# sdmiller/cpu_tsdf

Measured on AMD Instinct MI355X. Metric: integrateCloud throughput, Scene A turntable depth frames, 640x480 -> voxel grid, higher is better.
Workload: dtype f32

## Files before the change

### cpu_tsdf_amd/capi.py

```python
import ctypes as C
import os

import numpy as np

_HERE = os.path.dirname(os.path.abspath(__file__))
PRODUCT_LIB_PATH = os.path.join(_HERE, "lib", "libtsdf_hip.so")
TEST_LIB_PATH = os.path.join(_HERE, "lib", "libtsdf_hip_test.so")
LIB_PATH = os.environ.get("TSDF_HIP_LIB_PATH") or PRODUCT_LIB_PATH

OK, E_INVALID, E_NOMEM, E_HIP, E_NODEVICE, E_UNSUPPORTED, E_IO = range(7)
ALIGN_NO_POINTS, ALIGN_RANK_DEFICIENT = 7, 8
XFORM_PCL_SSE, XFORM_LEFT_TO_RIGHT = 0, 1
LAYOUT_AUTO, LAYOUT_F32W, LAYOUT_PACKED = 0, 1, 2
COLOR_RGB, COLOR_RGB_NORMALIZED, COLOR_LAB = 0, 1, 2


class TsdfParams(C.Structure):

    _fields_ = [
        ("res", C.c_int32 * 3),
        ("size", C.c_float * 3),
        ("max_dist_pos", C.c_float),
        ("max_dist_neg", C.c_float),
        ("max_weight", C.c_float),
        ("min_sensor_dist", C.c_float),
        ("max_sensor_dist", C.c_float),
        ("fx", C.c_double),
        ("fy", C.c_double),
        ("cx", C.c_double),
        ("cy", C.c_double),
        ("image_width", C.c_int32),
        ("image_height", C.c_int32),
        ("integrate_color", C.c_int32),
        ("xform_order", C.c_int32),
        ("z_begin", C.c_int32),
        ("z_end", C.c_int32),
        ("halo", C.c_int32),
        ("device", C.c_int32),
        ("layout", C.c_int32),
        ("color_mode", C.c_int32),
    ]


class TsdfVolMeta(C.Structure):

    _fields_ = [
        ("max_cell_size", C.c_float * 3),
        ("is_empty", C.c_int32),
        ("weight_by_depth", C.c_int32),
        ("weight_by_variance", C.c_int32),
        ("global_transform", C.c_double * 16),
    ]


BLOCK_FN = C.CFUNCTYPE(C.c_int, C.c_void_p, C.c_int, C.c_int, C.c_int, C.c_int, C.POINTER(C.c_float),
                       C.POINTER(C.c_float), C.POINTER(C.c_uint8))
HEADER_FN = C.CFUNCTYPE(C.c_int, C.c_void_p, C.POINTER(TsdfParams), C.POINTER(TsdfVolMeta))


class TsdfHipError(RuntimeError):
    def __init__(self, code, where, detail=""):
        self.code = code
        super().__init__(f"{where}: tsdf_hip error {code} ({detail})")


_lib = None

_f32p = C.POINTER(C.c_float)
_u8p = C.POINTER(C.c_uint8)
_u32p = C.POINTER(C.c_uint32)
_u64p = C.POINTER(C.c_uint64)
_f64p = C.POINTER(C.c_double)

SIGNATURES = {
    "tsdf_hip_default_params": (None, [C.POINTER(TsdfParams)]),
    "tsdf_hip_create": (C.c_int, [C.POINTER(TsdfParams), C.POINTER(C.c_void_p)]),
    "tsdf_hip_create_multi": (C.c_int, [C.POINTER(TsdfParams), C.POINTER(C.c_int32), C.c_int, C.POINTER(C.c_void_p)]),
    "tsdf_hip_slab_count": (C.c_int, [C.c_void_p]),
    "tsdf_hip_slab_info": (C.c_int, [C.c_void_p, C.c_int, C.POINTER(C.c_int32), C.POINTER(C.c_int32), C.POINTER(C.c_int32),
                                    C.POINTER(C.c_int32)]),
    "tsdf_hip_load_multi": (C.c_int, [C.c_char_p, C.POINTER(TsdfParams), C.POINTER(C.c_int32), C.c_int, C.POINTER(C.c_void_p),
                                     C.POINTER(TsdfParams), C.POINTER(TsdfVolMeta)]),
    "tsdf_hip_host_alloc": (C.c_int, [C.c_size_t, C.POINTER(C.c_void_p)]),
    "tsdf_hip_host_free": (C.c_int, [C.c_void_p]),
    "tsdf_hip_reset": (C.c_int, [C.c_void_p]),
    "tsdf_hip_destroy": (C.c_int, [C.c_void_p]),
    "tsdf_hip_set_stream": (C.c_int, [C.c_void_p, C.c_void_p]),
    "tsdf_hip_synchronize": (C.c_int, [C.c_void_p]),
    "tsdf_hip_integrate": (C.c_int, [C.c_void_p, _f32p, _u8p, _f32p, _u64p]),
    "tsdf_hip_integrate_async": (C.c_int, [C.c_void_p, _f32p, _u8p, _f32p]),
    "tsdf_hip_integrate_device": (C.c_int, [C.c_void_p, C.c_void_p, C.c_void_p, _f32p, _u64p]),
    "tsdf_hip_organize": (C.c_int, [C.c_void_p, _f32p, C.c_size_t, _u8p, C.c_size_t, C.c_size_t, C.c_float, C.c_int,
                                    _f64p, _f32p, _u8p, _u64p]),
    "tsdf_hip_integrate_staged": (C.c_int, [C.c_void_p, _f32p, _u64p]),
    "tsdf_hip_set_weighting": (C.c_int, [C.c_void_p, C.c_int, C.c_int]),
    "tsdf_hip_frame_begin": (C.c_int, [C.c_void_p, C.POINTER(_f32p), C.POINTER(_u8p)]),
    "tsdf_hip_frame_commit": (C.c_int, [C.c_void_p, _f32p]),
    "tsdf_hip_last_count_detail": (C.c_int, [C.c_void_p, _u64p]),
    "tsdf_hip_last_read_detail": (C.c_int, [C.c_void_p, _u64p]),
    "tsdf_hip_march_timing": (C.c_int, [C.c_void_p, _f32p, _u64p]),
    "tsdf_hip_march_stats": (C.c_int, [C.c_void_p, _u64p]),
    "tsdf_hip_raycast": (C.c_int, [C.c_void_p, _f32p, _f32p, C.c_int, _f32p]),
    "tsdf_hip_raycast_camera": (C.c_int, [C.c_void_p, _f32p, _f32p, C.c_int, _f64p, _f32p]),
    "tsdf_hip_raycast_begin": (C.c_int, [C.c_void_p, _f32p, _f32p, C.c_int, C.c_void_p]),
    "tsdf_hip_raycast_advance": (C.c_int, [C.c_void_p, _f32p, _f32p, C.c_int, C.c_int, C.c_int, C.c_void_p, C.c_void_p]),
    "tsdf_hip_raycast_advance_list": (C.c_int, [C.c_void_p, _f32p, _f32p, C.c_int, C.c_int, C.c_int, C.c_void_p, C.c_size_t]),
    "tsdf_hip_render_halo": (C.c_int, [C.POINTER(TsdfParams)]),
    "tsdf_hip_reference_cull_is_noop": (C.c_int, [C.POINTER(TsdfParams)]),
    "tsdf_hip_alloc_probe": (C.c_int, [C.c_void_p, _f32p, C.POINTER(C.c_int32)]),
    "tsdf_hip_sample": (C.c_int, [C.c_void_p, _f32p, C.c_size_t, _f32p, _f32p, _f32p, _u8p]),
    "tsdf_hip_lookup_rgb": (C.c_int, [C.c_void_p, _f32p, C.c_size_t, _u8p, _u8p]),
    "tsdf_hip_align_system": (C.c_int, [C.c_void_p, _f32p, C.c_size_t, _f64p, C.c_float, C.c_float, _f64p, _u8p, _f32p]),
    "tsdf_hip_align_system_device": (C.c_int, [C.c_void_p, C.c_void_p, C.c_size_t, _f64p, C.c_float, C.c_float, _f64p]),
    "tsdf_hip_align": (C.c_int, [C.c_void_p, _f32p, C.c_size_t, _f64p, C.c_float, C.c_float, C.c_int, C.c_double, _f64p,
                                 C.POINTER(C.c_int32), _f64p]),
    "tsdf_hip_align_stats": (C.c_int, [C.c_void_p, _u64p]),
    "tsdf_hip_march": (C.c_int, [C.c_void_p, C.c_float, C.c_int, _u64p]),
    "tsdf_hip_march_fetch": (C.c_int, [C.c_void_p, _f32p, _u8p, _u64p]),
    "tsdf_hip_march_fetch_device": (C.c_int, [C.c_void_p, C.c_void_p, C.c_void_p, C.c_void_p]),
    "tsdf_hip_mesh_cleanup": (C.c_int, [C.c_int, _f32p, C.c_uint64, _u32p, C.c_uint64, C.c_float, C.c_int, _u8p, _u64p]),
    "tsdf_hip_march_cleanup": (C.c_int, [C.c_void_p, C.c_float, C.c_int, _u64p]),
    "tsdf_hip_mesh_cleanup_stats": (C.c_int, [_u64p]),
    "tsdf_hip_mesh_flatten": (C.c_int, [C.c_int, _f32p, C.c_uint64, _u32p, C.c_uint64, C.c_float, _u32p, _u32p, _u64p, _u32p, _u64p]),
    "tsdf_hip_march_flatten": (C.c_int, [C.c_void_p, C.c_float, _u64p, _u64p]),
    "tsdf_hip_march_fetch_indexed": (C.c_int, [C.c_void_p, _f32p, _u8p, _u32p, _u64p]),
    "tsdf_hip_mesh_flatten_stats": (C.c_int, [_u64p]),
    "tsdf_hip_occupied": (C.c_int, [C.c_void_p, C.POINTER(C.c_int32), _u64p]),
    "tsdf_hip_occupied_fetch": (C.c_int, [C.c_void_p, C.POINTER(C.c_int32), _f32p, _f32p, _u8p]),
    "tsdf_hip_occupied_fetch_device": (C.c_int, [C.c_void_p, C.c_void_p, C.c_void_p, C.c_void_p, C.c_void_p]),
    "tsdf_hip_occupied_stats": (C.c_int, [C.c_void_p, _u64p]),
    "tsdf_hip_occupied_timing": (C.c_int, [C.c_void_p, _f32p]),
    "tsdf_hip_download": (C.c_int, [C.c_void_p] + [C.c_int] * 6 + [_f32p, _f32p, _u8p]),
    "tsdf_hip_upload": (C.c_int, [C.c_void_p] + [C.c_int] * 6 + [_f32p, _f32p, _u8p]),
    "tsdf_hip_download_color_state": (C.c_int, [C.c_void_p, C.c_int, C.c_int, C.c_int, _f32p]),
    "tsdf_hip_get_planes_device": (C.c_int, [C.c_void_p, C.c_int, C.c_int, C.c_void_p, C.c_void_p, C.c_void_p]),
    "tsdf_hip_set_planes_device": (C.c_int, [C.c_void_p, C.c_int, C.c_int, C.c_void_p, C.c_void_p, C.c_void_p]),
    "tsdf_hip_device_planes": (C.c_int, [C.c_void_p, C.POINTER(C.c_void_p), C.POINTER(C.c_void_p),
                                          C.POINTER(C.c_void_p), C.POINTER(C.c_int64),
                                          C.POINTER(C.c_int32), C.POINTER(C.c_int32)]),
    "tsdf_hip_layout": (C.c_int, [C.c_void_p]),
    "tsdf_hip_centers": (C.c_int, [C.c_void_p, C.c_int, _f32p]),
    "tsdf_hip_save": (C.c_int, [C.c_void_p, C.c_char_p, C.POINTER(TsdfVolMeta)]),
    "tsdf_hip_save_blocks": (C.c_int, [C.POINTER(TsdfParams), C.POINTER(TsdfVolMeta), C.c_char_p, BLOCK_FN, C.c_void_p]),
    "tsdf_hip_load_blocks": (C.c_int, [C.c_char_p, C.POINTER(TsdfParams), HEADER_FN, BLOCK_FN, C.c_void_p]),
    "tsdf_hip_load": (C.c_int, [C.c_char_p, C.POINTER(TsdfParams), C.POINTER(C.c_void_p), C.POINTER(TsdfParams),
                                C.POINTER(TsdfVolMeta)]),
    "tsdf_hip_error_string": (C.c_char_p, [C.c_int]),
    "tsdf_hip_last_error": (C.c_char_p, []),
    "tsdf_hip_device_count": (C.c_int, []),
    "tsdf_hip_abi_version": (C.c_int, []),
    "tsdf_hip_download_variance_state": (C.c_int, [C.c_void_p] + [C.c_int] * 6 + [_f32p, C.POINTER(C.c_int32)]),
    "tsdf_hip_upload_variance_state": (C.c_int, [C.c_void_p] + [C.c_int] * 6 + [_f32p, C.POINTER(C.c_int32)]),
    "tsdf_hip_set_reference_cull": (C.c_int, [C.c_void_p, _f32p]),
    "tsdf_hip_integrate_device2": (C.c_int, [C.c_void_p, C.c_void_p, C.c_void_p, _f32p, _f32p, C.c_void_p, C.c_void_p, _f32p, _f32p,
                                             _u64p, C.POINTER(C.c_int32)]),
    "tsdf_hip_set_frame_pairing": (C.c_int, [C.c_void_p, C.c_int]),
    "tsdf_hip_reference_cull_planes": (C.c_int, [C.POINTER(TsdfParams), _f64p, _f32p]),
    "tsdf_hip_last_launch_info": (C.c_int, [C.c_void_p, C.POINTER(C.c_int32)]),
    "tsdf_hip_multi_render_stats": (C.c_int, [C.c_void_p, _u64p]),
    "tsdf_hip_multi_link_stats": (C.c_int, [C.c_void_p, _u64p]),
    "tsdf_hip_multi_timing": (C.c_int, [C.c_void_p, C.c_int]),
    "tsdf_hip_multi_kernel_ms": (C.c_int, [C.c_void_p, C.c_int, _f32p, C.POINTER(C.c_int32)]),
}

TEST_SIGNATURES = {
    "tsdf_hip_selftest_checksum": (C.c_int, [C.c_void_p, _u64p]),
    "tsdf_hip_selftest_occupancy_mc": (C.c_int, [C.POINTER(C.c_int)]),
    "tsdf_hip_selftest_div_count": (C.c_int, [_f32p, C.POINTER(C.c_uint32), _f32p, _u8p, C.c_size_t]),
    "tsdf_hip_selftest_cvt_pk_u8": (C.c_int, [_f32p, C.c_size_t, C.POINTER(C.c_uint32)]),
    "tsdf_hip_selftest_rgb2lab": (C.c_int, [_u8p, C.c_size_t, _f32p]),
    "tsdf_hip_selftest_lab2rgb": (C.c_int, [_f32p, C.c_size_t, C.POINTER(C.c_uint32)]),
    "tsdf_hip_selftest_struct_oob": (C.c_int, [_f32p, C.c_int, C.c_int, C.c_int, C.c_int, C.POINTER(C.c_int32), C.POINTER(C.c_uint32), C.c_int]),
    "tsdf_hip_selftest_div_f32": (C.c_int, [_f32p, _f32p, _f32p, C.c_size_t]),
    "tsdf_hip_selftest_div_f64": (C.c_int, [_f64p, _f64p, _f64p, C.c_size_t]),
    "tsdf_hip_selftest_project": (C.c_int, [C.c_void_p, _f32p, C.c_size_t, C.POINTER(C.c_int32), C.POINTER(C.c_int32), _u8p]),
    "tsdf_hip_selftest_containing": (C.c_int, [C.c_void_p, _f32p, C.c_size_t, C.POINTER(C.c_int32)]),
    "tsdf_hip_selftest_sweep": (C.c_int, [C.c_void_p, _u64p, _u64p]),
    "tsdf_hip_selftest_read_sweep": (C.c_int, [C.c_void_p, C.c_int, _u64p, _u64p]),
    "tsdf_hip_set_tuning": (C.c_int, [C.c_char_p, C.c_int]),
    "tsdf_hip_selftest_block_flags": (C.c_int, [C.POINTER(TsdfParams), _f32p, C.c_int, C.c_int, _u8p]),
    "tsdf_hip_selftest_row_intervals": (C.c_int, [C.POINTER(TsdfParams), _f32p, _f32p, C.POINTER(C.c_uint32)]),
    "tsdf_hip_selftest_index_box": (C.c_int, [C.POINTER(TsdfParams), _f32p, C.POINTER(C.c_int32), C.POINTER(C.c_int32)]),
# ... 123 lines not shown
```

### cpu_tsdf_amd/csrc/tsdf_common.h

```cpp
#pragma once

#include <hip/hip_runtime.h>
#include <stdint.h>
#include <cmath>
#include <string>
#include <vector>

#include "tsdf_hip.h"

struct tsdf_hip_pipeline;
struct tsdf_hip_multi;

struct tsdf_hip_volume {
  tsdf_hip_multi *multi = nullptr;
  tsdf_params p;
  int device = 0;
  int nx = 0, ny = 0, nz = 0;
  int z_begin = 0, z_end = 0;
  int z_first = 0;
  int nz_alloc = 0;
  int64_t pitch = 0;
  int levels[3] = {0, 0, 0};
  float *d = nullptr, *w = nullptr;
  uint32_t *rgb = nullptr;
  uint8_t *k8 = nullptr;
  float *cn[4] = {nullptr, nullptr, nullptr, nullptr};
  float *lab_lut = nullptr;
  float4 *lab_img = nullptr;
  float *vm = nullptr;
  int32_t *vn = nullptr;
  int expf_fused_r = 0;
  float alloc_probe_ms[8] = {-1.f, -1.f, -1.f, -1.f, -1.f, -1.f, -1.f, -1.f};
  int alloc_tried = 0, alloc_chosen = 0;
  int packed = 0;
  unsigned kmax = 0;
  int weight_by_depth = 0, weight_by_variance = 0;
  float *ctr[3] = {nullptr, nullptr, nullptr};
  std::vector<float> h_ctr[3];
  float *frame_depth = nullptr;
  uint32_t *frame_bgra = nullptr;
  char *bounce = nullptr;
  hipEvent_t bounce_ev[2] = {nullptr, nullptr};
  bool bounce_busy[2] = {false, false};
  unsigned bounce_turn = 0;
  double *cam64 = nullptr;
  tsdf_hip_pipeline *pipe = nullptr;
  int frame_staged = 0;
  uint8_t *band = nullptr;
  int band_fx = 0, band_fy = 0;
  bool band_exact = false;
  int rest_state = 0;
  uint32_t rest_bits = 0;
  unsigned long long last_implied = 0, last_read_bytes = 0;
  bool last_implied_on = false;
  uint8_t *live = nullptr;
  size_t live_cap = 0;
  uint32_t *row_iv = nullptr;
  size_t row_iv_cap = 0;
  bool ctr_increasing[3] = {false, false, false};
  unsigned long long *counter = nullptr;
  unsigned long long last_observed = 0, last_changed_bytes = 0;
  bool ref_cull = false;
  float cull_planes[24] = {0};
  int last_launch[4] = {0, 0, 0, 0};
  bool pair_pending = false;
  bool pair_fused = false;
  unsigned long long pair_first_observed = 0, pair_first_changed = 0, pair_first_implied = 0, pair_first_read = 0;
  int count_slots = 0;
  bool count_ran = false;
  hipStream_t stream = nullptr;
  float *mc_verts = nullptr;
  uint8_t *mc_rgb = nullptr;
  uint64_t *mc_cell = nullptr;
  uint64_t mc_ntri = 0;
  size_t mc_cap = 0;
  bool mc_has_rgb = false;
  uint64_t *mc_keys = nullptr, *mc_vals = nullptr;
  size_t mc_cells_cap = 0;
  uint8_t *mc_need = nullptr;
  size_t mc_need_cap = 0;
  hipEvent_t mc_ev[4] = {nullptr, nullptr, nullptr, nullptr};
  float mc_ms[3] = {0.f, 0.f, 0.f};
  uint64_t mc_ncells = 0;
  uint64_t mc_d_bytes = 0;
  bool mc_skipped = false;
  hipEvent_t align_ev[2] = {nullptr, nullptr};
  uint64_t align_stats[4] = {0, 0, 0, 0};
  void *scratch = nullptr;
  size_t scratch_bytes = 0;
};

void tsdf_multi_free(tsdf_hip_volume *v);
int tsdf_multi_reset(tsdf_handle h);
int tsdf_multi_synchronize(tsdf_handle h);
int tsdf_multi_set_weighting(tsdf_handle h, int by_depth, int by_variance);
int tsdf_multi_set_reference_cull(tsdf_handle h, const float planes[24]);
int tsdf_multi_variance_block(tsdf_handle h, bool down, int x0, int y0, int z0, int nx, int ny, int nz, float *M, int32_t *nsample);
int tsdf_multi_integrate(tsdf_handle h, const float *depth, const uint8_t *bgra, const float T[12], uint64_t *n_observed,
                         bool asynchronous);
int tsdf_multi_integrate_device(tsdf_handle h, const float *d_depth, const uint32_t *d_bgra, const float T[12],
                                uint64_t *n_observed);
int tsdf_multi_organize(tsdf_handle h, const float *xyz, size_t xyz_stride, const uint8_t *bgra, size_t bgra_stride, size_t n,
                        float cloud_units, int zero_nans, const double world_to_cam[12], float *depth_out, uint8_t *bgra_out,
                        uint64_t *n_valid);
int tsdf_multi_integrate_staged(tsdf_handle h, const float T[12], uint64_t *n_observed);
int tsdf_multi_last_count_detail(tsdf_handle h, uint64_t out[2]);
int tsdf_multi_last_read_detail(tsdf_handle h, uint64_t out[3]);
int tsdf_multi_block(tsdf_handle h, bool down, int x0, int y0, int z0, int nx, int ny, int nz, float *d, float *w, uint8_t *rgb);
int tsdf_multi_sample(tsdf_handle h, const float *xyz, size_t n, float *val, float *grad, float *hess, uint8_t *ok);
int tsdf_multi_align_system(tsdf_handle h, const float *xyz, size_t n, const double vol_from_src[12], float min_weight, float r_max,
                            double out[29], uint8_t *used, float *xyz_vol);
int tsdf_multi_lookup_rgb(tsdf_handle h, const float *xyz, size_t n, uint8_t *rgb, uint8_t *found);
int tsdf_multi_raycast(tsdf_handle h, const float rot[9], const float origin[3], int downsample, const double *inv, float *out);
int tsdf_multi_march(tsdf_handle h, float w_min, int color_mode, uint64_t *n_tri);
int tsdf_multi_march_fetch(tsdf_handle h, float *verts, uint8_t *rgb, uint64_t *cell);
int tsdf_multi_march_timing(tsdf_handle h, float ms[3], uint64_t *n_cells);
int tsdf_multi_march_stats(tsdf_handle h, uint64_t out[4]);
tsdf_handle tsdf_multi_first(tsdf_handle h);
int tsdf_multi_flush(tsdf_handle h);
int tsdf_multi_set_frame_pairing(tsdf_handle h, int on);
int tsdf_multi_integrate_device2(tsdf_handle h, const float *da, const uint32_t *ca, const float TA[12], const float *planes_a, const float *db,
                                 const uint32_t *cb, const float TB[12], const float *planes_b, uint64_t *n_observed, int32_t *fused);
#define TSDF_NOT_ON_MULTI(h, what)                                                                          \
  do {                                                                                                      \
    if ((h) && (h)->multi) {                                                                                \
      tsdf_set_error(what " works on ONE slab handle; this handle is a multi-GPU set (tsdf_hip_create_multi)"); \
      return TSDF_HIP_E_UNSUPPORTED;                                                                        \
    }                                                                                                       \
  } while (0)

int tsdf_integrate_launch(tsdf_handle h, const float *d_depth, const uint32_t *d_bgra, const float T[12], bool count);
int tsdf_integrate_collect(tsdf_handle h, uint64_t *n_observed);
int tsdf_integrate_launch2(tsdf_handle h, const float *dA, const uint32_t *cA, const float TA[12], const float *planesA,
                           const float *dB, const uint32_t *cB, const float TB[12], const float *planesB, bool count, bool *fused);
int tsdf_integrate_collect2(tsdf_handle h, uint64_t n_observed[2]);

#define TSDF_MAX_SLABS 64
#define TSDF_RAY_FIN_INTS 9
unsigned tsdf_ray_list_share(int64_t n_rays, int rank, int world);
int tsdf_ray_list_begin(tsdf_handle s, const float rot[9], const float origin[3], int downsample, int rank, int world,
                        int32_t *d_list, unsigned *count);
int tsdf_ray_list_advance(tsdf_handle s, const float rot[9], const float origin[3], int downsample, int rank, int world,
                          int32_t *d_list, unsigned count, unsigned *d_incomplete);
int tsdf_ray_list_route(tsdf_handle s, const int32_t *d_list, unsigned count, int n_slab, const int *z_end,
                        unsigned *d_counters, int32_t *d_outbox, int32_t *d_finbox);
int tsdf_ray_deliver(tsdf_handle s, const int32_t *d_fin, unsigned count, float *d_out, int64_t n_pix, const double *inv);

void tsdf_set_error(const std::string &msg);
int tsdf_hip_fail(hipError_t e, const char *what, const char *file, int line);

#define TSDF_HIP_TRY(expr)                                              \
  do {                                                                  \
    hipError_t _e = (expr);                                             \
    if (_e != hipSuccess) return tsdf_hip_fail(_e, #expr, __FILE__, __LINE__); \
  } while (0)

struct TsdfDeviceScope {
  int prev = -1;
  hipError_t err;
  explicit TsdfDeviceScope(int dev) {
    err = hipGetDevice(&prev);
    if (err != hipSuccess || prev == dev)
      prev = -1;
    else
      err = hipSetDevice(dev);
  }
  ~TsdfDeviceScope() {
    if (prev >= 0) (void)hipSetDevice(prev);
  }
  TsdfDeviceScope(const TsdfDeviceScope &) = delete;
  TsdfDeviceScope &operator=(const TsdfDeviceScope &) = delete;
};
#define TSDF_ON_DEVICE(dev)          \
  TsdfDeviceScope _device_scope(dev); \
  TSDF_HIP_TRY(_device_scope.err)
int tsdf_pipeline_flush(tsdf_hip_volume *v);
#define TSDF_ENTER(h)                                  \
  TSDF_ON_DEVICE((h)->device);                         \
  if ((h)->pair_pending) {                             \
    const int _rc_flush = tsdf_pipeline_flush(h);      \
    if (_rc_flush) return _rc_flush;                   \
  }

void tsdf_build_centers(int res, float size, std::vector<float> &out, int *levels);
static inline void tsdf_lab_curve(float lut[256]) {
  for (int v = 0; v < 256; ++v) {
    float f = ((float)v / 255.);
    if (f > 0.0405)
      f = std::pow(((f + 0.055) / 1.055), 2.4);
    else
      f /= 12.92;
    f *= 100;
    lut[v] = f;
  }
}

static inline uint8_t tsdf_u8_of_float(float v) {
  const int i = (v > -2147483904.f && v < 2147483648.f) ? (int)v : (int)0x80000000;
  return (uint8_t)(i & 255);
}
static inline uint32_t tsdf_lab2rgb_host(float L, float A, float B) {
  float Y = (L + 16) / 116.;
  float X = A / 500. + Y;
  float Z = Y - (B / 200.);
  if (std::pow((double)X, 3.0) > 0.008856) X = std::pow((double)X, 3.0); else X = (X - 16 / 116.) / 7.787;
  if (std::pow((double)Y, 3.0) > 0.008856) Y = std::pow((double)Y, 3.0); else Y = (Y - 16 / 116.) / 7.787;
  if (std::pow((double)Z, 3.0) > 0.008856) Z = std::pow((double)Z, 3.0); else Z = (Z - 16 / 116.) / 7.787;
  X *= 95.047;
  Y *= 100.;
  Z *= 108.883;
  X /= 100;
  Y /= 100;
  Z /= 100;
  float rf = X * +3.2406 + Y * -1.5372 + Z * -0.4986;
  float gf = X * -0.9689 + Y * +1.8758 + Z * +0.0415;
  float bf = X * +0.0557 + Y * -0.2040 + Z * +1.0570;
  if (rf > 0.0031308) rf = 1.055 * std::pow(static_cast<double>(rf), 1. / 2.4) - 0.055; else rf *= 12.92;
  if (gf > 0.0031308) gf = 1.055 * std::pow(static_cast<double>(gf), 1. / 2.4) - 0.055; else gf *= 12.92;
  if (bf > 0.0031308) bf = 1.055 * std::pow(static_cast<double>(bf), 1. / 2.4) - 0.055; else bf *= 12.92;
  return (uint32_t)tsdf_u8_of_float(rf * 255) | ((uint32_t)tsdf_u8_of_float(gf * 255) << 8) | ((uint32_t)tsdf_u8_of_float(bf * 255) << 16);
}
void tsdf_lab2rgb_host_many(const float *L, const float *A, const float *B, size_t n, uint32_t *out);
int tsdf_lab_exact_colors(tsdf_hip_volume *v, const int64_t *d_idx, size_t n, uint32_t *host_rgb, bool write_plane);

static inline float tsdf_node_size(const tsdf_params &p, int axis) {
  const int r = p.res[0];
  const bool cubic_pow2 = r > 0 && (r & (r - 1)) == 0 && p.res[1] == r && p.res[2] == r;
  return cubic_pow2 ? p.size[0] : p.size[axis];
}
int tsdf_ensure_scratch(tsdf_hip_volume *v, size_t bytes);
int tsdf_to_host(tsdf_hip_volume *v, void *dst, const void *dev_src, size_t bytes);
int tsdf_to_device(tsdf_hip_volume *v, void *dev_dst, const void *src, size_t bytes);
void tsdf_pipeline_destroy(tsdf_hip_volume *v);

struct TsdfTuning {
  int rows_per_block;
  int blocks_per_cu;
  int fast_projection;
  int mc_flush_at;
  int mc_skip;
  int cull;
  int vol_chunk;
  int plain_kernel;
  int alloc_tries;
  int allin;
  int refcull_plain;
  int live_log2tx;
  int zfast;
  int fuse2;
  int implied_d;
  int pipe;
  int lab_chunk;
};
const TsdfTuning &tsdf_tuning();
int tsdf_vol_chunk();

struct PlaneView {
  const float *d, *w;
  const uint32_t *rgb;
  const uint8_t *k8;
  float wmax;
  unsigned kmax;
  int packed;
};

static inline PlaneView tsdf_plane_view(const tsdf_hip_volume *v) {
  return PlaneView{v->d, v->w, v->rgb, v->k8, v->p.max_weight, v->kmax, v->packed};
}

static __device__ __forceinline__ float tsdf_decode_w(unsigned k, float wmax) {
  const float kf = (float)k;
  return kf > wmax ? wmax : kf;
}

static __device__ __forceinline__ bool tsdf_encode_w(float w, float wmax, unsigned kmax, unsigned &k) {
  if (w == wmax) {
    k = kmax;
    return true;
  }
  if (w >= 0.f && w < (float)kmax && w == floorf(w)) {
    k = (unsigned)w;
    return true;
  }
  k = 0;
  return false;
}

static __device__ __forceinline__ float tsdf_load_w(const PlaneView &v, int64_t i) {
  if (!v.packed) return v.w[i];
  const unsigned k = v.rgb ? (v.rgb[i] >> 24) : (unsigned)v.k8[i];
  return tsdf_decode_w(k, v.wmax);
}

static __device__ __forceinline__ uint32_t tsdf_load_rgb(const PlaneView &v, int64_t i) {
  return v.rgb[i] & 0xffffffu;
}

static inline __host__ __device__ int64_t tsdf_index(int64_t pitch, int ny, int z_first, int x, int y,
                                                      int zg) {
  return ((int64_t)(zg - z_first) * ny + y) * pitch + x;
}
```

### cpu_tsdf_amd/csrc/tsdf_core.hip

```cpp
#include <math.h>

#include <string>
#include <stdlib.h>
#include <stdio.h>

#include <algorithm>
#include <thread>
#include <string.h>

#include <mutex>

#include "tsdf_common.h"
#include "tsdf_occupied.h"
#include "tsdf_meshpost.h"
#ifdef TSDF_HIP_TEST_HOOKS
#include "tsdf_hip_test.h"
#endif

static thread_local std::string g_last_error;

void tsdf_set_error(const std::string &msg) { g_last_error = msg; }

int tsdf_hip_fail(hipError_t e, const char *what, const char *file, int line) {
  char buf[512];
  snprintf(buf, sizeof buf, "%s:%d: %s -> %s", file, line, what, hipGetErrorString(e));
  g_last_error = buf;
  (void)hipGetLastError();
  return e == hipErrorOutOfMemory ? TSDF_HIP_E_NOMEM : TSDF_HIP_E_HIP;
}

extern "C" const char *tsdf_hip_last_error(void) { return g_last_error.c_str(); }

extern "C" const char *tsdf_hip_error_string(int code) {
  switch (code) {
    case TSDF_HIP_OK: return "ok";
    case TSDF_HIP_E_INVALID: return "invalid argument";
    case TSDF_HIP_E_NOMEM: return "out of device memory";
    case TSDF_HIP_E_HIP: return "HIP runtime error";
    case TSDF_HIP_E_NODEVICE: return "no HIP device";
    case TSDF_HIP_E_UNSUPPORTED: return "unsupported";
    case TSDF_HIP_E_IO: return "file error";
    case TSDF_HIP_ALIGN_NO_POINTS: return "alignment: no point passed the gate";
    case TSDF_HIP_ALIGN_RANK_DEFICIENT: return "alignment: the cloud does not constrain all six freedoms";
  }
  return "unknown";
}

static int env_int(const char *name, int dflt) {
  const char *e = getenv(name);
  return (e && *e) ? atoi(e) : dflt;
}

static TsdfTuning &tuning_storage() {
  static TsdfTuning t = {std::max(1, env_int("TSDF_HIP_ROWS_PER_BLOCK", 64)),
                         std::max(1, env_int("TSDF_HIP_BLOCKS_PER_CU", 8)),
                         env_int("TSDF_HIP_FAST_PROJECTION", -1), env_int("TSDF_HIP_MC_FLUSH_AT", 512), env_int("TSDF_HIP_MC_SKIP", 1),
                         env_int("TSDF_HIP_CULL", 1), std::max(1, env_int("TSDF_HIP_VOL_CHUNK", 256)),
                         env_int("TSDF_HIP_PLAIN_KERNEL", 0), env_int("TSDF_HIP_ALLOC_TRIES", 3), env_int("TSDF_HIP_ALLIN", 1),
                         env_int("TSDF_HIP_REFCULL_PLAIN", 0), env_int("TSDF_HIP_LIVE_LOG2TX", 5), env_int("TSDF_HIP_ZFAST", 1), env_int("TSDF_HIP_FUSE2", 1), env_int("TSDF_HIP_IMPLIED_D", 1),
                         env_int("TSDF_HIP_PIPE", 1), std::max(1, env_int("TSDF_HIP_LAB_CHUNK", 16 << 20))};
  return t;
}

const TsdfTuning &tsdf_tuning() { return tuning_storage(); }

int tsdf_vol_chunk() {
  const int live = env_int("TSDF_HIP_VOL_CHUNK", 0);
  return live > 0 ? live : tsdf_tuning().vol_chunk;
}

#ifdef TSDF_HIP_TEST_HOOKS
extern "C" int tsdf_hip_set_tuning(const char *name, int value) {
  if (!name) return TSDF_HIP_E_INVALID;
  TsdfTuning &t = tuning_storage();
  const std::string n(name);
  if (n == "rows_per_block")
    t.rows_per_block = std::max(1, value);
  else if (n == "blocks_per_cu")
    t.blocks_per_cu = std::max(1, value);
  else if (n == "fast_projection")
    t.fast_projection = value;
  else if (n == "mc_flush_at")
    t.mc_flush_at = value;
  else if (n == "mc_skip")
    t.mc_skip = value;
  else if (n == "cull")
    t.cull = value;
  else if (n == "vol_chunk")
    t.vol_chunk = std::max(1, value);
  else if (n == "plain_kernel")
    t.plain_kernel = value;
  else if (n == "alloc_tries")
    t.alloc_tries = std::max(1, value);
  else if (n == "allin")
    t.allin = value;
  else if (n == "refcull_plain")
    t.refcull_plain = value;
  else if (n == "fuse2")
    t.fuse2 = value;
  else if (n == "implied_d")
    t.implied_d = value;
  else if (n == "pipe")
    t.pipe = value;
  else if (n == "live_log2tx")
    t.live_log2tx = value;
  else if (n == "zfast")
    t.zfast = value;
  else if (n == "lab_chunk")
    t.lab_chunk = std::max(1, value);
  else
    return TSDF_HIP_E_INVALID;
  return TSDF_HIP_OK;
}
#endif

extern "C" int tsdf_hip_abi_version(void) { return TSDF_HIP_ABI_VERSION; }

extern "C" int tsdf_hip_host_alloc(size_t bytes, void **out) {
  if (!out || !bytes) return TSDF_HIP_E_INVALID;
  *out = nullptr;
  TSDF_HIP_TRY(hipHostMalloc(out, bytes, hipHostMallocPortable));
  return TSDF_HIP_OK;
}

extern "C" int tsdf_hip_host_free(void *p) {
  if (!p) return TSDF_HIP_OK;
  TSDF_HIP_TRY(hipHostFree(p));
  return TSDF_HIP_OK;
}

extern "C" int tsdf_hip_device_count(void) {
  int n = 0;
  if (hipGetDeviceCount(&n) != hipSuccess) {
    (void)hipGetLastError();
    return 0;
  }
  return n;
}

extern "C" void tsdf_hip_default_params(tsdf_params *p) {
  memset(p, 0, sizeof *p);
  p->res[0] = p->res[1] = p->res[2] = 512;
  p->size[0] = p->size[1] = p->size[2] = 3.0f;
  p->max_dist_pos = 0.03f;
  p->max_dist_neg = 0.03f;
  p->max_weight = 100.f;
  p->min_sensor_dist = 0.3f;
  p->max_sensor_dist = 3.0f;
  p->fx = p->fy = 525.;
  p->cx = 320;
  p->cy = 240;
  p->image_width = 640;
  p->image_height = 480;
  p->integrate_color = 0;
  p->xform_order = TSDF_XFORM_PCL_SSE;
  p->z_begin = p->z_end = 0;
  p->halo = 0;
  p->device = -1;
  p->layout = TSDF_LAYOUT_AUTO;
  p->color_mode = TSDF_COLOR_RGB;
}

static int ilog2_exact(int v) {
  if (v <= 0 || (v & (v - 1))) return -1;
  int l = 0;
  while ((1 << l) < v) ++l;
  return l;
}

void tsdf_build_centers(int res, float size, std::vector<float> &out, int *levels) {
  out.resize(res);
  const int L = ilog2_exact(res);
  *levels = L;
  if (L >= 0) {
    for (int i = 0; i < res; ++i) {
      float c = 0.f;
      float s = size;
      for (int l = L - 1; l >= 0; --l) {
        const float off = s / 4;
        c = ((i >> l) & 1) ? c + off : c - off;
        s = s / 2;
      }
      out[i] = c;
    }
  } else {
    const float off = size / 2.0;
    for (int i = 0; i < res; ++i) out[i] = (float)((i + 0.5) * size / (double)res - off);
  }
}

static __global__ void __launch_bounds__(256)
k_fill_u32(uint32_t *__restrict__ p, uint32_t value, int64_t n4 ) {
// ... 118 lines not shown
  return attr.type == hipMemoryTypeHost;
}

int tsdf_to_host(tsdf_hip_volume *v, void *dst, const void *dev_src, size_t bytes) {
  if (!bytes) return TSDF_HIP_OK;
  if (bytes >= (64u << 10) && is_pinned_host(dst)) {
    TSDF_HIP_TRY(hipMemcpyAsync(dst, dev_src, bytes, hipMemcpyDeviceToHost, v->stream));
    TSDF_HIP_TRY(hipStreamSynchronize(v->stream));
    return TSDF_HIP_OK;
  }
  int rc = bounce_ready(v);
  if (rc) return rc;
  const size_t chunks = (bytes + kBounceChunk - 1) / kBounceChunk;
  const unsigned turn = v->bounce_turn;
  v->bounce_turn += (unsigned)chunks;
  for (size_t k = 0; k <= chunks; ++k) {
    if (k < chunks) {
      const int slot = (int)((turn + k) & 1);
      if ((rc = bounce_wait(v, slot))) return rc;
      const size_t off = k * kBounceChunk, len = std::min(kBounceChunk, bytes - off);
      TSDF_HIP_TRY(hipMemcpyAsync(v->bounce + slot * kBounceChunk, (const char *)dev_src + off, len, hipMemcpyDeviceToHost,
                                  v->stream));
      TSDF_HIP_TRY(hipEventRecord(v->bounce_ev[slot], v->stream));
      v->bounce_busy[slot] = true;
    }
    if (k > 0) {
      const int slot = (int)((turn + k - 1) & 1);
      if ((rc = bounce_wait(v, slot))) return rc;
      const size_t off = (k - 1) * kBounceChunk, len = std::min(kBounceChunk, bytes - off);
      memcpy((char *)dst + off, v->bounce + slot * kBounceChunk, len);
    }
  }
  return TSDF_HIP_OK;
}

int tsdf_to_device(tsdf_hip_volume *v, void *dev_dst, const void *src, size_t bytes) {
  if (!bytes) return TSDF_HIP_OK;
  if (bytes >= (64u << 10) && is_pinned_host(src)) {
    TSDF_HIP_TRY(hipMemcpyAsync(dev_dst, src, bytes, hipMemcpyHostToDevice, v->stream));
    TSDF_HIP_TRY(hipStreamSynchronize(v->stream));
    return TSDF_HIP_OK;
  }
  int rc = bounce_ready(v);
  if (rc) return rc;
  const size_t chunks = (bytes + kBounceChunk - 1) / kBounceChunk;
  const unsigned turn = v->bounce_turn;
  v->bounce_turn += (unsigned)chunks;
  for (size_t k = 0; k < chunks; ++k) {
    const int slot = (int)((turn + k) & 1);
    if ((rc = bounce_wait(v, slot))) return rc;
    const size_t off = k * kBounceChunk, len = std::min(kBounceChunk, bytes - off);
    memcpy(v->bounce + slot * kBounceChunk, (const char *)src + off, len);
    TSDF_HIP_TRY(hipMemcpyAsync((char *)dev_dst + off, v->bounce + slot * kBounceChunk, len, hipMemcpyHostToDevice, v->stream));
    TSDF_HIP_TRY(hipEventRecord(v->bounce_ev[slot], v->stream));
    v->bounce_busy[slot] = true;
  }
  return TSDF_HIP_OK;
}

static void free_volume(tsdf_hip_volume *v) {
  if (!v) return;
  if (v->multi) tsdf_multi_free(v);
  TsdfDeviceScope scope(v->device);
  tsdf_pipeline_destroy(v);
  if (v->d) (void)hipFree(v->d);
  if (v->w) (void)hipFree(v->w);
  if (v->rgb) (void)hipFree(v->rgb);
  if (v->k8) (void)hipFree(v->k8);
  for (int c = 0; c < 4; ++c)
    if (v->cn[c]) (void)hipFree(v->cn[c]);
  if (v->vm) (void)hipFree(v->vm);
  if (v->vn) (void)hipFree(v->vn);
  if (v->lab_lut) (void)hipFree(v->lab_lut);
  if (v->lab_img) (void)hipFree(v->lab_img);
  for (int a = 0; a < 3; ++a)
    if (v->ctr[a]) (void)hipFree(v->ctr[a]);
  if (v->frame_depth) (void)hipFree(v->frame_depth);
  if (v->bounce) (void)hipHostFree(v->bounce);
  for (int i = 0; i < 2; ++i)
    if (v->bounce_ev[i]) (void)hipEventDestroy(v->bounce_ev[i]);
  if (v->cam64) (void)hipFree(v->cam64);
  if (v->live) (void)hipFree(v->live);
  if (v->row_iv) (void)hipFree(v->row_iv);
  if (v->band) (void)hipFree(v->band);
  if (v->counter) (void)hipFree(v->counter);
  if (v->mc_verts) (void)hipFree(v->mc_verts);
  if (v->mc_rgb) (void)hipFree(v->mc_rgb);
  if (v->mc_cell) (void)hipFree(v->mc_cell);
  if (v->mc_keys) (void)hipFree(v->mc_keys);
  if (v->mc_vals) (void)hipFree(v->mc_vals);
  if (v->mc_need) (void)hipFree(v->mc_need);
  for (int i = 0; i < 4; ++i)
    if (v->mc_ev[i]) (void)hipEventDestroy(v->mc_ev[i]);
  for (int i = 0; i < 2; ++i)
    if (v->align_ev[i]) (void)hipEventDestroy(v->align_ev[i]);
  if (v->scratch) (void)hipFree(v->scratch);
  delete v;
}

struct PlaneSet {
  float *d = nullptr, *w = nullptr;
  uint32_t *rgb = nullptr;
  uint8_t *k8 = nullptr;
};

static __global__ void __launch_bounds__(256)
k_probe_rmw(uint4 *__restrict__ a, uint4 *__restrict__ b, uint4 *__restrict__ c, int64_t n4, unsigned zero) {
  typedef unsigned v4u __attribute__((ext_vector_type(4)));
  v4u *pa = reinterpret_cast<v4u *>(a), *pb = reinterpret_cast<v4u *>(b), *pc = reinterpret_cast<v4u *>(c);
  for (int64_t i = (int64_t)blockIdx.x * blockDim.x + threadIdx.x; i < n4; i += (int64_t)gridDim.x * blockDim.x) {
    v4u x = __builtin_nontemporal_load(pa + i);
    x ^= zero;
    __builtin_nontemporal_store(x, pa + i);
    if (b) {
      v4u y = __builtin_nontemporal_load(pb + i);
      y ^= zero;
      __builtin_nontemporal_store(y, pb + i);
    }
    if (c) {
      v4u z = __builtin_nontemporal_load(pc + i);
      z ^= zero;
      __builtin_nontemporal_store(z, pc + i);
    }
  }
}

static void release_planes(PlaneSet &s) {
  if (s.d) (void)hipFree(s.d);
  if (s.w) (void)hipFree(s.w);
  if (s.rgb) (void)hipFree(s.rgb);
  if (s.k8) (void)hipFree(s.k8);
  s = PlaneSet();
}

static float probe_planes(const PlaneSet &s, int64_t n, hipStream_t stream) {
  hipEvent_t e0 = nullptr, e1 = nullptr;
  if (hipEventCreate(&e0) != hipSuccess || hipEventCreate(&e1) != hipSuccess) return -1.f;
  float ms = -1.f;
  const int64_t n4 = n / 4;
  const unsigned grid = 256u * (unsigned)tsdf_tuning().blocks_per_cu;
  bool ok = true;
  for (int pass = 0; pass < 2 && ok; ++pass) {
    ok &= hipEventRecord(e0, stream) == hipSuccess;
    hipLaunchKernelGGL(k_probe_rmw, dim3(grid), dim3(256), 0, stream, (uint4 *)s.d, (uint4 *)s.w, (uint4 *)s.rgb, n4, 0u);
    ok &= hipGetLastError() == hipSuccess;
    ok &= hipEventRecord(e1, stream) == hipSuccess;
    ok &= hipEventSynchronize(e1) == hipSuccess;
    if (ok) ok &= hipEventElapsedTime(&ms, e0, e1) == hipSuccess;
  }
  (void)hipEventDestroy(e0);
  (void)hipEventDestroy(e1);
  return ok ? ms : -1.f;
}

extern "C" int tsdf_hip_reference_cull_is_noop(const tsdf_params *p) {
  if (!p || !(p->fx > 0.0) || !(p->fy > 0.0) || p->image_width <= 0 || p->image_height <= 0) return 0;
  if (!(p->max_sensor_dist > 0.f) || !(p->max_sensor_dist < 1e15f)) return 0;
  const double W = p->image_width, H = p->image_height;
  const double th = tan(1.1 * atan(0.5 * W / p->fx)) * (1.0 - 1e-5), tv = tan(1.1 * atan(0.5 * H / p->fy)) * (1.0 - 1e-5);
  if (!(th > 0.0) || !(tv > 0.0)) return 0;
  return (p->cx + 1.0) / p->fx <= th && (W - p->cx) / p->fx <= th && (p->cy + 1.0) / p->fy <= tv && (H - p->cy) / p->fy <= tv;
}

extern "C" int tsdf_hip_reference_cull_planes(const tsdf_params *p, const double trans[16], float planes[24]) {
  if (!p || !trans || !planes) return TSDF_HIP_E_INVALID;
  struct V3 { float v[3]; };
// ... 94 lines not shown
  auto bail = [&](int code) {
    free_volume(v);
    return code;
  };
#define TRY_OR_BAIL(expr)                                                  \
  do {                                                                     \
    hipError_t _e = (expr);                                                \
    if (_e != hipSuccess) return bail(tsdf_hip_fail(_e, #expr, __FILE__, __LINE__)); \
  } while (0)
  auto alloc_planes = [&](PlaneSet &s) -> hipError_t {
    hipError_t e = hipMalloc(&s.d, n * sizeof(float));
    if (e == hipSuccess && !v->packed) e = hipMalloc(&s.w, n * sizeof(float));
    if (e == hipSuccess && p->integrate_color) e = hipMalloc(&s.rgb, n * sizeof(uint32_t));
    if (e == hipSuccess && v->packed && !p->integrate_color) e = hipMalloc(&s.k8, n);
    if (e != hipSuccess) release_planes(s);
    return e;
  };
  PlaneSet best;
  TRY_OR_BAIL(alloc_planes(best));
  {
    const size_t plane_bytes = (size_t)n * (4 + (v->packed ? 0 : 4) + (p->integrate_color ? 4 : 0) + (v->packed && !p->integrate_color ? 1 : 0));
    const int tries = plane_bytes >= ((size_t)4 << 30) ? std::max(1, tsdf_tuning().alloc_tries) : 1;
    float best_ms = tries > 1 ? probe_planes(best, n, v->stream) : -1.f;
    v->alloc_probe_ms[0] = best_ms;
    v->alloc_tried = 1;
    const double swept = (double)n * (4 + (v->packed ? 0 : 4) + (p->integrate_color ? 4 : 0));
    auto rate_tbps = [&](float ms) { return ms > 0.f ? 2.0 * swept / ((double)ms * 1e9) : 0.0; };
    for (int t = 1; t < std::min(8, 2 * tries) && best_ms > 0.f && tries > 1; ++t) {
      if (rate_tbps(best_ms) >= 5.55) break;
      if (t >= tries && rate_tbps(best_ms) >= 5.15) break;
      size_t free_b = 0, total_b = 0;
      if (hipMemGetInfo(&free_b, &total_b) != hipSuccess || free_b < plane_bytes + ((size_t)2 << 30)) break;
      PlaneSet cand;
      if (alloc_planes(cand) != hipSuccess) {
        (void)hipGetLastError();
        break;
      }
      const float ms = probe_planes(cand, n, v->stream);
      v->alloc_probe_ms[t < 8 ? t : 7] = ms;
      v->alloc_tried = t + 1;
      if (ms > 0.f && ms < best_ms) {
        release_planes(best);
        best = cand;
        best_ms = ms;
        v->alloc_chosen = t;
      } else {
        release_planes(cand);
      }
    }
  }
  v->d = best.d;
  v->w = best.w;
  v->rgb = best.rgb;
  v->k8 = best.k8;
  if (rgbn)
    for (int c = 0; c < (lab ? 3 : 4); ++c) TRY_OR_BAIL(hipMalloc(&v->cn[c], n * sizeof(float)));
  if (lab) {
    float lut[256];
    tsdf_lab_curve(lut);
    TRY_OR_BAIL(hipMalloc(&v->lab_lut, sizeof lut));
    TRY_OR_BAIL(hipMemcpy(v->lab_lut, lut, sizeof lut, hipMemcpyHostToDevice));
    TRY_OR_BAIL(hipMalloc(&v->lab_img, (size_t)p->image_width * p->image_height * sizeof(float4)));
  }
  for (int a = 0; a < 3; ++a) {
    tsdf_build_centers(p->res[a], tsdf_node_size(*p, a), v->h_ctr[a], &v->levels[a]);
    v->ctr_increasing[a] = true;
    for (size_t i = 1; i < v->h_ctr[a].size(); ++i) v->ctr_increasing[a] &= v->h_ctr[a][i - 1] < v->h_ctr[a][i];
    std::vector<float> padded(v->h_ctr[a]);
    padded.resize((size_t)p->res[a] + 4, NAN);
    TRY_OR_BAIL(hipMalloc(&v->ctr[a], padded.size() * sizeof(float)));
    TRY_OR_BAIL(hipMemcpy(v->ctr[a], padded.data(), padded.size() * sizeof(float), hipMemcpyHostToDevice));
  }
  const size_t npx = (size_t)p->image_width * p->image_height;
  TRY_OR_BAIL(hipMalloc(&v->frame_depth, 2 * npx * sizeof(float)));
  v->frame_bgra = reinterpret_cast<uint32_t *>(v->frame_depth + npx);
  {
    const double cam[4] = {p->fx, p->fy, p->cx, p->cy};
    TRY_OR_BAIL(hipMalloc(&v->cam64, sizeof cam));
    TRY_OR_BAIL(hipMemcpy(v->cam64, cam, sizeof cam, hipMemcpyHostToDevice));
  }
  v->band_fx = (v->nx + 63) / 64;
  v->band_fy = (v->ny + 3) / 4;
  TRY_OR_BAIL(hipMalloc(&v->band, (size_t)v->band_fx * v->band_fy * v->nz_alloc));
  TRY_OR_BAIL(hipMalloc(&v->counter, 4096 * sizeof(unsigned long long)));
  TRY_OR_BAIL(hipMemset(v->counter, 0, 4096 * sizeof(unsigned long long)));
#undef TRY_OR_BAIL
  rc = tsdf_hip_reset(v);
  if (rc != TSDF_HIP_OK) return bail(rc);
  *out = v;
  return TSDF_HIP_OK;
}

extern "C" int tsdf_hip_reset(tsdf_handle h) {
  if (!h) return TSDF_HIP_E_INVALID;
  if (h->multi) return tsdf_multi_reset(h);
  TSDF_ENTER(h);
  const int64_t n = h->pitch * h->ny * h->nz_alloc;
  const float minus_one = -1.f;
  uint32_t bits;
  memcpy(&bits, &minus_one, 4);
  int rc = fill_u32(h, h->d, bits, n);
  if (rc) return rc;
  if (h->w) rc = fill_u32(h, h->w, 0u, n);
  if (rc) return rc;
  if (h->k8) TSDF_HIP_TRY(hipMemsetAsync(h->k8, 0, (size_t)n, h->stream));
  if (h->rgb) rc = fill_u32(h, h->rgb, 0u, n);
  if (rc) return rc;
  for (int c = 0; c < 4 && !rc; ++c)
    if (h->cn[c]) rc = fill_u32(h, h->cn[c], 0u, n);
  if (rc) return rc;
  if (h->vm) rc = fill_u32(h, reinterpret_cast<float *>(h->vm), 0u, n);
  if (!rc && h->vn) rc = fill_u32(h, reinterpret_cast<float *>(h->vn), 0u, n);
  if (rc) return rc;
  TSDF_HIP_TRY(hipMemsetAsync(h->band, 0, (size_t)h->band_fx * h->band_fy * h->nz_alloc, h->stream));
  h->band_exact = true;
  h->rest_state = 0;
  TSDF_HIP_TRY(hipStreamSynchronize(h->stream));
  return TSDF_HIP_OK;
}

extern "C" int tsdf_hip_destroy(tsdf_handle h) {
  if (!h) return TSDF_HIP_E_INVALID;
  TsdfDeviceScope scope(h->device);
  (void)hipStreamSynchronize(h->stream);
  tsdf_occupied_release(h);
  tsdf_meshpost_release(h);
  free_volume(h);
  return TSDF_HIP_OK;
}

extern "C" int tsdf_hip_set_stream(tsdf_handle h, void *hip_stream) {
  if (!h) return TSDF_HIP_E_INVALID;
  TSDF_NOT_ON_MULTI(h, "tsdf_hip_set_stream (a stream belongs to one device)");
  {
    TSDF_ENTER(h);
  }
  h->stream = (hipStream_t)hip_stream;
  return TSDF_HIP_OK;
}

extern "C" int tsdf_hip_synchronize(tsdf_handle h) {
  if (!h) return TSDF_HIP_E_INVALID;
  if (h->multi) return tsdf_multi_synchronize(h);
  TSDF_ENTER(h);
  TSDF_HIP_TRY(hipStreamSynchronize(h->stream));
  return TSDF_HIP_OK;
}

extern "C" int tsdf_hip_centers(tsdf_handle h, int axis, float *out) {
  if (!h || axis < 0 || axis > 2 || !out) return TSDF_HIP_E_INVALID;
  memcpy(out, h->h_ctr[axis].data(), h->h_ctr[axis].size() * sizeof(float));
  return TSDF_HIP_OK;
}

extern "C" int tsdf_hip_alloc_probe(tsdf_handle h, float ms[8], int32_t *chosen) {
  if (!h) return 0;
  const tsdf_hip_volume *s = h->multi ? tsdf_multi_first(h) : h;
  if (ms)
    for (int i = 0; i < 8; ++i) ms[i] = s->alloc_probe_ms[i];
  if (chosen) *chosen = s->alloc_chosen;
  return s->alloc_tried;
}

extern "C" int tsdf_hip_layout(tsdf_handle h) {
  return !h ? -1 : (h->packed ? TSDF_LAYOUT_PACKED : TSDF_LAYOUT_F32W);
}

extern "C" int tsdf_hip_device_planes(tsdf_handle h, float **d, float **w, uint32_t **rgb, int64_t *pitch,
// ... 420 lines not shown
```

### cpu_tsdf_amd/csrc/tsdf_integrate.hip

```cpp
#include <limits.h>
#include <string.h>
#include <math.h>

#include <algorithm>
#include <cmath>

#include "tsdf_common.h"
#include "tsdf_div.h"
#include "tsdf_buffer.h"
#ifdef TSDF_HIP_TEST_HOOKS
#include "tsdf_hip_test.h"
#endif

#ifndef TSDF_COLOR_PK
#define TSDF_COLOR_PK 2
#endif

typedef float f2 __attribute__((ext_vector_type(2)));
typedef float f4 __attribute__((ext_vector_type(4)));

struct IntegrateArgs {
  float m[12];
  float fxf, fyf, cxf, cyf;
  float hb_u, hb_v;
  float hb_max;
  unsigned kcap, kinc;
  int hinge_fixed;
  int neg_in_window;
  unsigned kmax;
  int wmax_is_int;
  float zmin, zmax;
  float zlo;
  float pos, neg;
  float wmax;
  float pos_over_neg;
  int W, H;
  int ny;
  int plane_rows;
  int qpr;
  int z_global0;
  int zl0;
  int log2TX, TX, TY;
  int rpb;
  unsigned bgra_off;
  int expf_fused_r;
  int ref_cull;
  float cull[24];
  int band_fx, band_fy;
  int implied_d;
  int x_abs0, y_abs0;
  int zfast;
  int64_t pitch;
};

static __device__ __forceinline__ int project_exact(const IntegrateArgs &a, const double *__restrict__ cam,
                                                    float gx, float gy, float gz) {
  const Rcp64 rz = rcp64_prepare((double)gz);
  const int u = (int)(div64((double)gx * cam[0], rz) + cam[2]);
  const int v = (int)(div64((double)gy * cam[1], rz) + cam[3]);
  const bool in = (unsigned)u < (unsigned)a.W && (unsigned)v < (unsigned)a.H;
  return in ? v * a.W + u : -1;
}

template <bool ALLIN = false>
static __device__ __forceinline__ int project_fast(const IntegrateArgs &a, float gx, float gy, float gz,
                                                   bool &ambiguous, uint32_t *margin = nullptr) {
  const float y = __builtin_amdgcn_rcpf(gz);
  const float ru = __builtin_fmaf(gx * a.fxf, y, a.cxf);
  const float rv = __builtin_fmaf(gy * a.fyf, y, a.cyf);
  const int u = (int)ru, v = (int)rv;
  if (ALLIN) {
    *margin = min(__float_as_uint(__builtin_amdgcn_fractf(ru)), __float_as_uint(__builtin_amdgcn_fractf(rv)));
    ambiguous = false;
    return (int)__umul24((unsigned)v, (unsigned)a.W) + u;
  }
  const bool cert = __builtin_amdgcn_fractf(ru) > a.hb_u && __builtin_amdgcn_fractf(rv) > a.hb_v;
  ambiguous = !cert;
  const bool in = (unsigned)u < (unsigned)a.W && (unsigned)v < (unsigned)a.H;
  return in ? (int)__umul24((unsigned)v, (unsigned)a.W) + u : -1;
}

template <int ORDER>
static __device__ __forceinline__ void project_quad_allin(const IntegrateArgs &a, const float (&m)[12], const double *__restrict__ cam,
                                                          const f4 cxv, const f4 ytv, const float (&zt)[3], int (&pix)[4],
                                                          float (&gzs)[4]) {
  const f2 cxa = {cxv.x, cxv.y}, cxb = {cxv.z, cxv.w};
  const float yt[3] = {ytv.x, ytv.y, ytv.z};
  f2 ga[3], gb[3];
#pragma unroll
  for (int q = 0; q < 3; ++q) {
    if (ORDER == TSDF_XFORM_PCL_SSE) {
      ga[q] = cxa * m[4 * q] + yt[q];
      gb[q] = cxb * m[4 * q] + yt[q];
    } else {
      ga[q] = ((cxa * m[4 * q] + yt[q]) + zt[q]) + m[4 * q + 3];
      gb[q] = ((cxb * m[4 * q] + yt[q]) + zt[q]) + m[4 * q + 3];
    }
  }
  const f2 ya = {__builtin_amdgcn_rcpf(ga[2].x), __builtin_amdgcn_rcpf(ga[2].y)};
  const f2 yb = {__builtin_amdgcn_rcpf(gb[2].x), __builtin_amdgcn_rcpf(gb[2].y)};
  const f2 cxf2 = {a.cxf, a.cxf}, cyf2 = {a.cyf, a.cyf};
  const f2 rua = __builtin_elementwise_fma(ga[0] * a.fxf, ya, cxf2), rub = __builtin_elementwise_fma(gb[0] * a.fxf, yb, cxf2);
  const f2 rva = __builtin_elementwise_fma(ga[1] * a.fyf, ya, cyf2), rvb = __builtin_elementwise_fma(gb[1] * a.fyf, yb, cyf2);
  const float ru[4] = {rua.x, rua.y, rub.x, rub.y}, rv[4] = {rva.x, rva.y, rvb.x, rvb.y};
  gzs[0] = ga[2].x, gzs[1] = ga[2].y, gzs[2] = gb[2].x, gzs[3] = gb[2].y;
  uint32_t fu[4], fv[4];
#pragma unroll
  for (int j = 0; j < 4; ++j) {
    fu[j] = __float_as_uint(__builtin_amdgcn_fractf(ru[j]));
    fv[j] = __float_as_uint(__builtin_amdgcn_fractf(rv[j]));
    pix[j] = (int)__umul24((unsigned)(int)rv[j], (unsigned)a.W) + (int)ru[j];
  }
  const uint32_t hb = __float_as_uint(a.hb_max);
  const uint32_t least = min(min(min(fu[0], fv[0]), min(min(fu[1], fv[1]), fu[2])), min(min(fv[2], fu[3]), fv[3]));
  if (!(least > hb)) {
    const float gx[4] = {ga[0].x, ga[0].y, gb[0].x, gb[0].y}, gy[4] = {ga[1].x, ga[1].y, gb[1].x, gb[1].y};
#pragma unroll
    for (int j = 0; j < 4; ++j)
      if (!(min(fu[j], fv[j]) > hb)) pix[j] = project_exact(a, cam, gx[j], gy[j], gzs[j]);
  }
}

static __device__ const uint64_t k_exp2f_tab[32] = {
    0x3ff0000000000000ull, 0x3fefd9b0d3158574ull, 0x3fefb5586cf9890full, 0x3fef9301d0125b51ull, 0x3fef72b83c7d517bull,
    0x3fef54873168b9aaull, 0x3fef387a6e756238ull, 0x3fef1e9df51fdee1ull, 0x3fef06fe0a31b715ull, 0x3feef1a7373aa9cbull,
    0x3feedea64c123422ull, 0x3feece086061892dull, 0x3feebfdad5362a27ull, 0x3feeb42b569d4f82ull, 0x3feeab07dd485429ull,
    0x3feea47eb03a5585ull, 0x3feea09e667f3bcdull, 0x3fee9f75e8ec5f74ull, 0x3feea11473eb0187ull, 0x3feea589994cce13ull,
    0x3feeace5422aa0dbull, 0x3feeb737b0cdc5e5ull, 0x3feec49182a3f090ull, 0x3feed503b23e255dull, 0x3feee89f995ad3adull,
    0x3feeff76f2fb5e47ull, 0x3fef199bdd85529cull, 0x3fef3720dcef9069ull, 0x3fef5818dcfba487ull, 0x3fef7c97337b9b5full,
    0x3fefa4afa2a490daull, 0x3fefd0765b6e4540ull};

static __device__ float tsdf_expf_glibc(float x, bool fused_r) {
  const uint32_t ix = __float_as_uint(x), abstop = (ix >> 20) & 0x7ffu;
  if (abstop >= (0x42b00000u >> 20)) {
    if (ix == 0xff800000u) return 0.f;
    if (abstop >= (0x7f800000u >> 20)) return x + x;
// ... 154 lines not shown
#endif
#ifndef TSDF_EARLY_VOXEL_LOADS
#define TSDF_EARLY_VOXEL_LOADS 2
#endif

#ifndef TSDF_KTAB
#define TSDF_KTAB 0
#endif
#ifndef TSDF_LEAN_K
#define TSDF_LEAN_K 1
#endif
#ifndef TSDF_SWAR_K
#define TSDF_SWAR_K 1
#endif
#ifndef TSDF_LEAN_BAND
#define TSDF_LEAN_BAND 1
#endif
#ifndef TSDF_AMB_UNROLL
#define TSDF_AMB_UNROLL 1
#endif
#ifndef TSDF_PROJ_F2
#define TSDF_PROJ_F2 1
#endif
struct __attribute__((aligned(16))) KEntry {
  float w;
  float y;
  float hy;
  uint32_t k1;
};
static __device__ __forceinline__ KEntry tsdf_ktab_entry(const IntegrateArgs &a, unsigned k) {
  KEntry e;
  e.w = __builtin_fminf((float)k, a.wmax);
  e.y = rcp32_prepare((float)(k + 1u)).y;
  e.hy = TSDF_COLOR_PK == 2 ? __builtin_fmaf(0.5f, e.y, -0.5f) : 0.5f * e.y;
  e.k1 = min(k << 24, a.kcap) + a.kinc;
  return e;
}
#ifndef TSDF_SKIP_FIXED_HINGE
#define TSDF_SKIP_FIXED_HINGE 1
#endif
#ifndef TSDF_EXP_NO_STORE
#define TSDF_EXP_NO_STORE 0
#endif
#ifndef TSDF_EXP_NO_GATHER
#define TSDF_EXP_NO_GATHER 0
#endif
#ifndef TSDF_EXP_NO_VLOAD
#define TSDF_EXP_NO_VLOAD 0
#endif
#if TSDF_EXP_NO_VLOAD && TSDF_EARLY_VOXEL_LOADS
#error "TSDF_EXP_NO_VLOAD declares the voxel words itself: build it with -DTSDF_EARLY_VOXEL_LOADS=0 (tools/ab_bound.sh does)"
#endif
#if !TSDF_GUARD_ON_RESULT && TSDF_EARLY_VOXEL_LOADS
#error "TSDF_GUARD_ON_RESULT=0 tests the numerator d0 * w0 + dn BEFORE unread distance words are rebuilt from the counts, and with TSDF_EARLY_VOXEL_LOADS those words have no initial value: build that A/B with -DTSDF_EARLY_VOXEL_LOADS=0"
#endif
#ifndef TSDF_GATHER_AUX
#define TSDF_GATHER_AUX 0
#endif
#ifndef TSDF_WPE_MAX
#define TSDF_WPE_MAX 8
#endif
#ifndef TSDF_NO_BAND
#define TSDF_NO_BAND 0
#endif
#ifndef TSDF_BAND_PER_WAVE
#define TSDF_BAND_PER_WAVE 1
#endif
#if TSDF_BAND_PER_WAVE
#define TSDF_BAND_DECL                                                                                     \
  __shared__ __attribute__((aligned(16))) uint8_t s_band_sets[4][1024];                                    \
  reinterpret_cast<u4 *>(&s_band_sets[0][0])[tid] = (u4){0u, 0u, 0u, 0u}
#define TSDF_BAND(i) s_band_sets[threadIdx.x >> 6][i]
#define TSDF_BAND_SYNC() ((void)0)
#define TSDF_BAND_FIRST ((int)(tid & 63u))
#define TSDF_BAND_STEP 64
#else
#define TSDF_BAND_DECL                                                          \
  __shared__ __attribute__((aligned(16))) uint8_t s_band[1024 + 64];            \
  reinterpret_cast<uint32_t *>(s_band)[tid] = 0u, s_band[1024 + (tid & 63u)] = 0
#define TSDF_BAND(i) s_band[i]
#define TSDF_BAND_SYNC() __syncthreads()
#define TSDF_BAND_FIRST ((int)tid)
#define TSDF_BAND_STEP 256
#endif
#ifndef TSDF_RECOMPUTE_PX
#define TSDF_RECOMPUTE_PX 1
#endif
#ifndef TSDF_WPE_PACKED
#define TSDF_WPE_PACKED 7
#endif
#ifndef TSDF_WPE_PACKED_COLOR
#define TSDF_WPE_PACKED_COLOR 8
#endif
#define TSDF_WPE_OF(ORDER, COLOR, FASTPROJ, COUNT, PACKED, ALLIN) \
  ((ALLIN) && !(COUNT) && (PACKED) && (COLOR) && (FASTPROJ) ? TSDF_WPE_PACKED_COLOR : (ALLIN) && !(COUNT) && ((PACKED) || !(COLOR)) ? TSDF_WPE_PACKED : TSDF_WPE_GENERAL)
#ifndef TSDF_WPE_GENERAL
#define TSDF_WPE_GENERAL 7
#endif
#ifndef TSDF_PHASE_TIMER
#define TSDF_PHASE_TIMER 0
#endif
#if TSDF_PHASE_TIMER
#define TSDF_NPHASE 16
__device__ unsigned long long g_phase[1024 * TSDF_NPHASE];
static __device__ __forceinline__ uint32_t tsdf_clock_lo() {
  uint64_t t;
  asm volatile("s_memtime %0\n\ts_waitcnt lgkmcnt(0)" : "=s"(t)::"memory");
  return (uint32_t)t;
}
#define TSDF_NACC 9
#define PT_DECL                                                   \
  uint32_t pt_acc[TSDF_NACC];                                     \
  _Pragma("unroll") for (int i_ = 0; i_ < TSDF_NACC; ++i_) asm volatile("v_mov_b32 %0, 0" : "=v"(pt_acc[i_])); \
  const unsigned pt_blk = (blockIdx.x + blockIdx.y * gridDim.x + blockIdx.z * gridDim.x * gridDim.y) & 1023u; \
  uint32_t pt_prev = tsdf_clock_lo();                             \
  const uint32_t pt_t0 = pt_prev
#define PT_MARK(k)                           \
  do {                                       \
    const uint32_t pt_now = tsdf_clock_lo(); \
    pt_acc[k] += pt_now - pt_prev;           \
    pt_prev = pt_now;                        \
  } while (0)
                    \

#define PT_MARK_OUT(k)                                                                                 \
  do {                                                                                                 \
    const uint32_t pt_now = tsdf_clock_lo();                                                           \
    if ((threadIdx.x & 63u) == 0u) atomicAdd(&g_phase[pt_blk * TSDF_NPHASE + (k)], (unsigned long long)(pt_now - pt_prev)); \
    pt_prev = pt_now;                                                                                  \
  } while (0)
#define PT_COUNT(k) pt_acc[k] += 1u
#define PT_DEP4(a_, b_, c_, d_) asm volatile("" ::"v"(a_), "v"(b_), "v"(c_), "v"(d_) : "memory")
#define PT_DEP1(a_) asm volatile("" ::"v"(a_) : "memory")
#define PT_FLUSH()                                                                                       \
  do {                                                                                                   \
    const uint32_t pt_now = tsdf_clock_lo();                                                             \
    if ((threadIdx.x & 63u) == 0u) {                                                                     \
      atomicAdd(&g_phase[pt_blk * TSDF_NPHASE + 15], (unsigned long long)(pt_now - pt_t0));              \
      _Pragma("unroll") for (int i_ = 0; i_ < TSDF_NACC; ++i_)                                           \
          atomicAdd(&g_phase[pt_blk * TSDF_NPHASE + i_], (unsigned long long)pt_acc[i_]);                \
    }                                                                                                    \
  } while (0)
#else
#define PT_DECL
#define PT_MARK(k)
#define PT_MARK_OUT(k)
#define PT_COUNT(k)
#define PT_DEP4(a_, b_, c_, d_)
#define PT_DEP1(a_)
#define PT_FLUSH()
#endif
template <int ORDER, bool COLOR, bool FASTPROJ, bool COUNT, bool PACKED, bool ALLIN = false, bool LIVE = false>
static __global__ void __launch_bounds__(256) __attribute__((amdgpu_waves_per_eu(TSDF_WPE_OF(ORDER, COLOR, FASTPROJ, COUNT, PACKED, ALLIN) < TSDF_WPE_MAX ? TSDF_WPE_OF(ORDER, COLOR, FASTPROJ, COUNT, PACKED, ALLIN) : TSDF_WPE_MAX, TSDF_WPE_MAX)))
k_integrate(const IntegrateArgs a, float *__restrict__ D, float *__restrict__ Wt, uint32_t *__restrict__ RGB,
            uint8_t *__restrict__ K8, const float *__restrict__ depth, const double *__restrict__ cam,
            const float *__restrict__ ctrx, const float *__restrict__ ctry, const float *__restrict__ ctrz,
            unsigned long long *__restrict__ n_obs, const uint8_t *__restrict__ live, uint8_t *__restrict__ band,
            const uint32_t *__restrict__ row_iv) {
  static_assert(!(ALLIN && LIVE), "the ALLIN instance knows no row intervals");
  const BlockCoords bc = tsdf_block_coords(a.zfast);
  PT_DECL;
  bool strad = false;
  if (LIVE) {
    const unsigned flag = live[bc.bx + bc.gdx * (bc.by + bc.gdy * bc.bz)];
    if (flag == 0u) return;
    strad = flag == 2u;
  }
  const unsigned tid = threadIdx.x;
#if TSDF_KTAB
  __shared__ KEntry s_tab[PACKED ? 256 : 1];
#else
  __shared__ f2 s_rcp[256];
#endif
  __shared__ f4 s_yt[256];
  constexpr bool F2 = TSDF_PROJ_F2 && ALLIN && FASTPROJ;
  constexpr bool LEAN_K1 = TSDF_LEAN_K && !TSDF_KTAB && TSDF_COLOR_PK == 2 && PACKED && COLOR;
  __shared__ f4 s_cx[F2 ? 256 : 1];
  __shared__ uint32_t s_iv[LIVE ? 256 : 1];
  TSDF_BAND_DECL;
#if TSDF_KTAB
  if (PACKED) s_tab[tid] = tsdf_ktab_entry(a, tid);
#else
  if (PACKED) {
    const KEntry e = tsdf_ktab_entry(a, tid);
    s_rcp[tid] = (f2){e.y, e.hy};
  }
#endif
  {
    const int yy = (int)bc.by * a.rpb * a.TY + (int)tid;
    {
      const float cy_ = ctry[yy < a.ny ? yy : a.ny - 1], cz_ = ctrz[a.z_global0 + (int)bc.bz];
      f4 t = {0.f, 0.f, 0.f, 0.f};
#pragma unroll
      for (int q = 0; q < 3; ++q)
        t[q] = ORDER == TSDF_XFORM_PCL_SSE ? cy_ * a.m[4 * q + 1] + (cz_ * a.m[4 * q + 2] + a.m[4 * q + 3]) : a.m[4 * q + 1] * cy_;
      s_yt[tid] = t;
    }
    if (F2) {
      const int xq_ = (int)bc.bx * a.TX + (int)(tid & (unsigned)(a.TX - 1));
      if (xq_ < a.qpr) s_cx[tid] = *reinterpret_cast<const f4 *>(ctrx + xq_ * 4);
    }
    if (LIVE && strad) s_iv[tid] = yy < a.ny ? row_iv[(int64_t)bc.bz * a.ny + yy] : 0u;
  }
  __shared__ uint8_t s_bin[PACKED ? 1024 : 1];
  if (PACKED && a.implied_d) tsdf_flags_before(a, bc, band, s_bin, tid);
  __syncthreads();
  const uint64_t quiet = PACKED && a.implied_d ? tsdf_quiet_passes(a, s_bin, tid) : 0ull;
  PT_MARK_OUT(9);
  const int tx = (int)(tid & (unsigned)(a.TX - 1));
  const int ty = (int)(tid >> a.log2TX);
  const int xq = (int)bc.bx * a.TX + tx;
  const int zl = (int)bc.bz;
  const Rcp32 rneg = rcp32_prepare(a.neg);
  unsigned cnt = 0, chg = 0, imp = 0, rdb = 0;
  const int row0 = (int)bc.by * a.rpb * a.TY;
  const int rows = min(a.rpb * a.TY, a.ny - row0);
  const int64_t e0 = ((int64_t)(a.zl0 + zl) * a.plane_rows + row0) * a.pitch;
  const unsigned span = (unsigned)rows * (unsigned)a.pitch;
  const rsrc_t rsD = make_rsrc(D + e0, span * 4u);
  const rsrc_t rsW = make_rsrc(PACKED ? D : Wt + e0, PACKED ? 0u : span * 4u);
  const rsrc_t rsC = make_rsrc(COLOR ? RGB + e0 : (uint32_t *)D, COLOR ? span * 4u : 0u);
  const rsrc_t rsK = make_rsrc(PACKED && !COLOR ? K8 + e0 : (uint8_t *)D, PACKED && !COLOR ? span : 0u);
  const unsigned npix = (unsigned)a.W * (unsigned)a.H;
  const rsrc_t rsF = make_rsrc(depth, COLOR ? a.bgra_off + npix * 4u : npix * 4u);
  const i4_rsrc rsFi = make_rsrc_2d(depth, 4u, 0xffffffffu);
  if (xq < a.qpr) {
    const int x4 = xq * 4;
    const float cz = ctrz[a.z_global0 + zl];
    const float4 cx4 = *reinterpret_cast<const float4 *>(ctrx + x4);
    const float cxs[4] = {cx4.x, cx4.y, cx4.z, cx4.w};
    float px_[4][3], zt[3];
#pragma unroll
    for (int r = 0; r < 3; ++r) {
#pragma unroll
      for (int j = 0; j < 4; ++j) px_[j][r] = cxs[j] * a.m[4 * r];
      zt[r] = ORDER == TSDF_XFORM_PCL_SSE ? cz * a.m[4 * r + 2] + a.m[4 * r + 3] : a.m[4 * r + 2] * cz;
    }
    const unsigned voff = (unsigned)(ty * (int)a.pitch + x4) * 4u;
    const unsigned row_step = (unsigned)a.TY * (unsigned)a.pitch * 4u;
#if TSDF_EARLY_VOXEL_LOADS
    bool pred_obs = true;
#endif
    for (int r = 0; r < a.rpb; ++r) {
      const int y = row0 + ty + r * a.TY;
      if (y >= a.ny) break;
      unsigned iv_lo = 0u, iv_len = 0u;
      if (LIVE && strad) {
        const uint32_t iv = s_iv[ty + r * a.TY];
        iv_lo = iv & 0xffffu, iv_len = iv >> 16;
        if (!((unsigned)(x4 + 3) - iv_lo < iv_len + 3u)) continue;
      }
      const unsigned soff = (unsigned)r * row_step;
      const f4 ytv = s_yt[ty + r * a.TY];
      const float yt[3] = {ytv.x, ytv.y, ytv.z};
#if TSDF_RECOMPUTE_PX
      float px[4][3];
      if constexpr (!F2) {
        float cxr[4] = {cxs[0], cxs[1], cxs[2], cxs[3]};
#pragma unroll
        for (int j = 0; j < 4; ++j) asm volatile("" : "+v"(cxr[j]));
#pragma unroll
        for (int q = 0; q < 3; ++q)
#pragma unroll
          for (int j = 0; j < 4; ++j) px[j][q] = cxr[j] * a.m[4 * q];
      }
#else
      const float (&px)[4][3] = px_;
#endif
      auto transform = [&](int j, int q) -> float {
        if (ORDER == TSDF_XFORM_PCL_SSE) return px[j][q] + yt[q];
        return ((px[j][q] + yt[q]) + zt[q]) + a.m[4 * q + 3];
      };
      int pix[4];
      float gzs[4];
      bool any = false, lowz = false;
      if constexpr (F2) {
        asm volatile("" ::: "memory");
        project_quad_allin<ORDER>(a, a.m, cam, s_cx[tid], ytv, zt, pix, gzs);
        PT_DEP4(pix[0], pix[1], pix[2], pix[3]);
        PT_MARK(0);
      } else {
      unsigned amb_mask = 0;
      uint32_t margin[4] = {0u, 0u, 0u, 0u};
#pragma unroll
      for (int j = 0; j < 4; ++j) {
        const float gx = transform(j, 0), gy = transform(j, 1), gz = transform(j, 2);
        const bool in = ALLIN || (gz > a.zlo && !(gz > a.zmax) && (!LIVE || !strad || (unsigned)(x4 + j) - iv_lo < iv_len));
        gzs[j] = gz;
        if (!ALLIN) lowz |= in && gz < 0x1p-14f;
        int p;
        if (FASTPROJ) {
          bool amb;
          p = project_fast<ALLIN>(a, gx, gy, gz, amb, &margin[j]);
          if (amb && in) amb_mask |= 1u << j;
        } else {
          p = project_exact(a, cam, gx, gy, in ? gz : 1.f);
        }
        pix[j] = in ? p : -1;
        any |= in;
      }
      if (!ALLIN && !any) continue;
      if (ALLIN && FASTPROJ) {
        const uint32_t hb = __float_as_uint(a.hb_max);
        if (!(min(min(margin[0], margin[1]), min(margin[2], margin[3])) > hb)) {
#pragma unroll
          for (int j = 0; j < 4; ++j)
            if (!(margin[j] > hb)) amb_mask |= 1u << j;
        }
      }
#if TSDF_AMB_UNROLL
      if (FASTPROJ && amb_mask) {
#pragma unroll
        for (int j = 0; j < 4; ++j)
          if (amb_mask >> j & 1u) pix[j] = project_exact(a, cam, transform(j, 0), transform(j, 1), transform(j, 2));
      }
#else
      while (FASTPROJ && amb_mask) {
        const int j = __builtin_ctz(amb_mask);
        amb_mask &= amb_mask - 1;
        float g[3];
#pragma unroll
        for (int q = 0; q < 3; ++q)
          g[q] = j == 0 ? transform(0, q) : j == 1 ? transform(1, q) : j == 2 ? transform(2, q) : transform(3, q);
        const int p = project_exact(a, cam, g[0], g[1], g[2]);
        if (j == 0) pix[0] = p;
        if (j == 1) pix[1] = p;
        if (j == 2) pix[2] = p;
        if (j == 3) pix[3] = p;
      }
#endif
      }
#if TSDF_EARLY_VOXEL_LOADS
      constexpr bool EARLY = PACKED;
      const bool d_read = !PACKED || !(r < 64 && (quiet >> r & 1ull));
      u4 d4;
      asm volatile("" : "=v"(d4));
      u4 w4 = {0u, 0u, 0u, 0u}, c4 = {0u, 0u, 0u, 0u};
      uint32_t k4 = 0u;
      const bool ask_early = EARLY && (TSDF_EARLY_VOXEL_LOADS != 2 || pred_obs);
      if (ask_early) {
        if (d_read) d4 = bload128(rsD, voff, soff);
        if (COLOR) c4 = bload128(rsC, voff, soff);
        if (!COLOR) k4 = bload32(rsK, voff >> 2, soff >> 2);
        if (COUNT) rdb += (d_read ? 16u : 0u) + (COLOR ? 16u : 4u);
      }
#endif
      float zs[4];
      uint32_t cs[4] = {0u, 0u, 0u, 0u};
#pragma unroll
      for (int j = 0; j < 4; ++j) {
        if (TSDF_EXP_NO_GATHER) {
          zs[j] = 1e3f + (float)(pix[j] & 1);
          cs[j] = 0x00406080u + (unsigned)pix[j];
        } else if (ALLIN) {
          zs[j] = __uint_as_float(tsdf_struct_buffer_load_u32(rsFi, pix[j], 0, 0, TSDF_GATHER_AUX));
          if (COLOR) cs[j] = tsdf_struct_buffer_load_u32(rsFi, pix[j], 0, (int)a.bgra_off, TSDF_GATHER_AUX);
        } else {
          zs[j] = __uint_as_float(bload32(rsF, (unsigned)pix[j] << 2, 0u));
          if (COLOR) cs[j] = bload32(rsF, (unsigned)pix[j] << 2, a.bgra_off);
        }
      }
      PT_MARK(1);
      PT_DEP4(zs[0], zs[1], zs[2], zs[3]);
      PT_MARK(2);
      float dn[4], raw[4];
      bool act[4];
      any = false;
      bool any_div = false;
#pragma unroll
      for (int j = 0; j < 4; ++j) {
        raw[j] = zs[j] - gzs[j];
        act[j] = (ALLIN || pix[j] >= 0) && raw[j] >= -a.neg;
        dn[j] = a.pos_over_neg;
        any |= act[j];
        if (!TSDF_LEAN_BAND) any_div |= act[j] && !(raw[j] > a.pos);
      }
      if (TSDF_LEAN_BAND) {
        if (__builtin_fminf(__builtin_fminf(raw[0], raw[1]), __builtin_fminf(raw[2], raw[3])) <= a.pos) {
#pragma unroll
          for (int j = 0; j < 4; ++j) any_div |= act[j] && !(raw[j] > a.pos);
        }
      }
      if (COLOR) asm volatile("" ::"v"(cs[0]), "v"(cs[1]), "v"(cs[2]), "v"(cs[3]));
#if TSDF_EARLY_VOXEL_LOADS
      if (EARLY) {
        if (COLOR)
          asm volatile("" ::"v"(d4), "v"(c4));
        else
          asm volatile("" ::"v"(d4), "v"(k4));
      }
      const bool asked_early = ask_early;
      pred_obs = any;
#endif
      PT_MARK(3);
      if (!any) continue;
      PT_COUNT(8);
#if TSDF_EARLY_VOXEL_LOADS == 2
      if (EARLY && !asked_early) {
        if (d_read) d4 = bload128(rsD, voff, soff);
        if (COLOR) c4 = bload128(rsC, voff, soff);
        if (!COLOR) k4 = bload32(rsK, voff >> 2, soff >> 2);
        if (COUNT) rdb += (d_read ? 16u : 0u) + (COLOR ? 16u : 4u);
      }
#endif
      if (any_div) {
#pragma unroll
        for (int j = 0; j < 4; ++j) dn[j] = raw[j] > a.pos ? a.pos_over_neg : div32_fast(raw[j], rneg);
      }
      if (lowz || !a.neg_in_window) {
        asm volatile("");
#pragma unroll
        for (int j = 0; j < 4; ++j)
          if (act[j] && !(raw[j] > a.pos)) dn[j] = raw[j] / a.neg;
      }
#if TSDF_EXP_NO_VLOAD
      const uint32_t hb_ = __float_as_uint(a.pos_over_neg);
      const u4 d4 = {hb_, hb_, hb_, hb_};
      u4 w4 = {0u, 0u, 0u, 0u}, c4 = {(unsigned)r << 24, (unsigned)r << 24, (unsigned)r << 24, (unsigned)r << 24};
      uint32_t k4 = 0u;
      const bool d_read = true;
#else
#if !TSDF_EARLY_VOXEL_LOADS
      constexpr bool EARLY = false;
      const bool d_read = !PACKED || !(r < 64 && (quiet >> r & 1ull));
      u4 d4 = {0u, 0u, 0u, 0u};
      u4 w4 = {0u, 0u, 0u, 0u}, c4 = {0u, 0u, 0u, 0u};
      uint32_t k4 = 0u;
#endif
      if (!EARLY) {
        if (d_read) d4 = bload128(rsD, voff, soff);
        if (!PACKED) w4 = bload128(rsW, voff, soff);
        if (COLOR) c4 = bload128(rsC, voff, soff);
        if (PACKED && !COLOR) k4 = bload32(rsK, voff >> 2, soff >> 2);
        if (COUNT) rdb += (d_read ? 16u : 0u) + (!PACKED ? 16u : 0u) + (COLOR ? 16u : 0u) + (PACKED && !COLOR ? 4u : 0u);
      }
#endif
      PT_MARK(4);
      if (COLOR) PT_DEP4(c4.x, c4.y, c4.z, c4.w); else PT_DEP1(k4);
      PT_MARK(5);
      uint32_t d0u[4] = {d4.x, d4.y, d4.z, d4.w};
      const uint32_t c0[4] = {c4.x, c4.y, c4.z, c4.w};
      const uint32_t w0u[4] = {w4.x, w4.y, w4.z, w4.w};
      float d0[4], w0[4];
      uint32_t kw[4];
      float dv[4], wv[4];
      uint32_t cv[4], k1[4];
#if TSDF_KTAB
      float ky[4];
#endif
      float khy[4] = {0.f, 0.f, 0.f, 0.f};
#pragma unroll
      for (int j = 0; j < 4; ++j) {
        d0[j] = __uint_as_float(d0u[j]);
        w0[j] = __uint_as_float(w0u[j]);
        kw[j] = 0u;
        k1[j] = 0u;
        if (PACKED) {
          kw[j] = COLOR ? c0[j] : (k4 << (24 - 8 * j));
#if TSDF_KTAB
          const KEntry e = s_tab[kw[j] >> 24];
          w0[j] = e.w, ky[j] = e.y, khy[j] = e.hy, k1[j] = e.k1;
#else
          if (TSDF_LEAN_K && ALLIN) {
// ... 93 lines not shown
#pragma unroll
        for (int j = 0; j < 4; ++j) {
          dv[j] = d0[j];
          wv[j] = w0[j];
          cv[j] = c0[j] & 0xffffffu;
          add_observation_ieee<COLOR>(dv[j], wv[j], cv[j], dn[j], cs[j], a.wmax);
          if (COLOR) cv[j] |= k1[j] & 0xff000000u;
        }
      }
      PT_DEP4(dv[0], dv[1], cv[0], cv[1]);
      PT_MARK(6);
      uint32_t diff_w = 0u, diff_c = 0u, k4n = 0u;
      uint32_t wn_u[4];
      const uint32_t c_before[4] = {c0[0], c0[1], c0[2], c0[3]};
      if (d_touched) {
        uint32_t diff_d = 0u, dn_u[4];
#pragma unroll
        for (int j = 0; j < 4; ++j) {
          dn_u[j] = act[j] ? __float_as_uint(dv[j]) : d0u[j];
          diff_d |= dn_u[j] ^ d0u[j];
          if (COUNT) chg += dn_u[j] != d0u[j] ? 4u : 0u;
        }
        if (diff_d && !TSDF_EXP_NO_STORE) bstore128(rsD, voff, soff, (u4){dn_u[0], dn_u[1], dn_u[2], dn_u[3]});
      }
#pragma unroll
      for (int j = 0; j < 4; ++j) {
        if (PACKED && !COLOR && !TSDF_SWAR_K) k4n |= (act[j] ? k1[j] : (kw[j] & 0xff000000u)) >> (24 - 8 * j);
        wn_u[j] = act[j] ? __float_as_uint(wv[j]) : w0u[j];
        cv[j] = act[j] ? cv[j] : c0[j];
        diff_w |= wn_u[j] ^ w0u[j];
        diff_c |= cv[j] ^ c0[j];
        cnt += act[j] ? 1u : 0u;
        if (COUNT && PACKED) imp += act[j] && !d_read ? 1u : 0u;
        if (COUNT)
          chg += (!PACKED && wn_u[j] != w0u[j] ? 4u : 0u) + (COLOR && cv[j] != c_before[j] ? 4u : 0u);
      }
      if (PACKED && !COLOR && TSDF_SWAR_K) {
        const uint32_t km2 = a.kmax * 0x00010001u;
        const uint32_t te = ((k4 & 0x00ff00ffu) | 0x01000100u) - km2, to = (((k4 >> 8) & 0x00ff00ffu) | 0x01000100u) - km2;
        const uint32_t lt = ((~te >> 8) & 0x00010001u) | (((~to >> 8) & 0x00010001u) << 8);
        const uint32_t actb = (act[0] ? 0x00000001u : 0u) | (act[1] ? 0x00000100u : 0u) | (act[2] ? 0x00010000u : 0u) | (act[3] ? 0x01000000u : 0u);
        k4n = k4 + (lt & actb);
      }
      if (COUNT && PACKED && !COLOR) chg += (unsigned)__popc(((k4n ^ k4) | ((k4n ^ k4) >> 1) | ((k4n ^ k4) >> 2) | ((k4n ^ k4) >> 3) |
                                                            ((k4n ^ k4) >> 4) | ((k4n ^ k4) >> 5) | ((k4n ^ k4) >> 6) | ((k4n ^ k4) >> 7)) & 0x01010101u);
      if (!PACKED && diff_w) bstore128(rsW, voff, soff, (u4){wn_u[0], wn_u[1], wn_u[2], wn_u[3]});
      if (TSDF_EXP_NO_STORE) {
        if ((cv[0] ^ cv[1] ^ cv[2] ^ cv[3]) == 0x12345678u) bstore32(rsD, voff, soff, cv[0] ^ diff_w);
      } else
      if (COLOR && diff_c) bstore128(rsC, voff, soff, (u4){cv[0], cv[1], cv[2], cv[3]});
      if (PACKED && !COLOR && k4n != k4) bstore32(rsK, voff >> 2, soff >> 2, k4n);
      PT_MARK(7);
    }
  }
  PT_MARK_OUT(10);
  if (!TSDF_NO_BAND && band) {
    TSDF_BAND_SYNC();
    const int lf = max(0, a.log2TX - 4), fxb = 1 << lf;
    const int yg0 = (a.y_abs0 + row0) >> 2, yg1 = (a.y_abs0 + row0 + max(rows, 1) - 1) >> 2;
    const int xc0 = (a.x_abs0 + (int)bc.bx * a.TX * 4) >> 6;
    const int n_fl = (yg1 - yg0 + 1) << lf;
    for (int i = TSDF_BAND_FIRST; i < n_fl; i += TSDF_BAND_STEP) {
      const int yg = yg0 + (i >> lf), xc = xc0 + (i & (fxb - 1));
      if (TSDF_BAND(i) && yg < a.band_fy && xc < a.band_fx) band[((int64_t)(a.zl0 + zl) * a.band_fy + yg) * a.band_fx + xc] = 1;
    }
  }
  PT_MARK_OUT(12);
  PT_FLUSH();
  if (COUNT) {
    __shared__ unsigned s_cnt, s_chg, s_imp, s_rdb;
    if (tid == 0) s_cnt = s_chg = s_imp = s_rdb = 0;
    __syncthreads();
    if (cnt) atomicAdd(&s_cnt, cnt);
    if (chg) atomicAdd(&s_chg, chg);
    if (imp) atomicAdd(&s_imp, imp);
    if (rdb) atomicAdd(&s_rdb, rdb);
    __syncthreads();
    if (tid == 0 && (s_cnt || s_rdb)) {
      const unsigned b = bc.bx + bc.by * bc.gdx + bc.bz * bc.gdx * bc.gdy;
      if (s_cnt) atomicAdd(n_obs + (b & 1023u), (unsigned long long)s_cnt);
      if (s_chg) atomicAdd(n_obs + 1024u + (b & 1023u), (unsigned long long)s_chg);
      if (s_imp) atomicAdd(n_obs + 2048u + (b & 1023u), (unsigned long long)s_imp);
      if (s_rdb) atomicAdd(n_obs + 3072u + (b & 1023u), (unsigned long long)s_rdb);
    }
  }
}

#ifndef TSDF_WPE_PIPE
#define TSDF_WPE_PIPE 8
#endif
struct PipeRow {
  float gz[4];
  uint32_t z[4];
  uint32_t k4;
  u4 d4;
};

template <int ORDER, bool COUNT>
static __global__ void __launch_bounds__(256) __attribute__((amdgpu_waves_per_eu(TSDF_WPE_PIPE < TSDF_WPE_MAX ? TSDF_WPE_PIPE : TSDF_WPE_MAX, TSDF_WPE_MAX)))
k_integrate_p(const IntegrateArgs a, float *__restrict__ D, uint8_t *__restrict__ K8, const float *__restrict__ depth,
              const double *__restrict__ cam, const float *__restrict__ ctrx, const float *__restrict__ ctry,
              const float *__restrict__ ctrz, unsigned long long *__restrict__ n_obs, uint8_t *__restrict__ band) {
  const BlockCoords bc = tsdf_block_coords(a.zfast);
  const unsigned tid = threadIdx.x;
  __shared__ f2 s_rcp[256];
  __shared__ f4 s_yt[256];
  __shared__ f4 s_cx[256];
  __shared__ uint8_t s_bin[1024];
  TSDF_BAND_DECL;
  {
    const KEntry e = tsdf_ktab_entry(a, tid);
    s_rcp[tid] = (f2){e.y, e.hy};
    const int yy = (int)bc.by * a.rpb * a.TY + (int)tid;
    const float cy_ = ctry[yy < a.ny ? yy : a.ny - 1], cz_ = ctrz[a.z_global0 + (int)bc.bz];
    f4 t = {0.f, 0.f, 0.f, 0.f};
#pragma unroll
    for (int q = 0; q < 3; ++q)
      t[q] = ORDER == TSDF_XFORM_PCL_SSE ? cy_ * a.m[4 * q + 1] + (cz_ * a.m[4 * q + 2] + a.m[4 * q + 3]) : a.m[4 * q + 1] * cy_;
    s_yt[tid] = t;
    const int xq_ = (int)bc.bx * a.TX + (int)(tid & (unsigned)(a.TX - 1));
    if (xq_ < a.qpr) s_cx[tid] = *reinterpret_cast<const f4 *>(ctrx + xq_ * 4);
  }
  if (a.implied_d) tsdf_flags_before(a, bc, band, s_bin, tid);
  __syncthreads();
  const uint64_t quiet = a.implied_d ? tsdf_quiet_passes(a, s_bin, tid) : 0ull;
  const int tx = (int)(tid & (unsigned)(a.TX - 1));
  const int ty = (int)(tid >> a.log2TX);
  const int xq = (int)bc.bx * a.TX + tx;
  const int zl = (int)bc.bz;
  const Rcp32 rneg = rcp32_prepare(a.neg);
  unsigned cnt = 0, chg = 0, imp = 0, rdb = 0;
  const int row0 = (int)bc.by * a.rpb * a.TY;
  const int rows = min(a.rpb * a.TY, a.ny - row0);
  const int64_t e0 = ((int64_t)(a.zl0 + zl) * a.plane_rows + row0) * a.pitch;
  const unsigned span = (unsigned)rows * (unsigned)a.pitch;
  const rsrc_t rsD = make_rsrc(D + e0, span * 4u);
  const rsrc_t rsK = make_rsrc(K8 + e0, span);
  const i4_rsrc rsFi = make_rsrc_2d(depth, 4u, 0xffffffffu);
  const uint32_t pbits = __float_as_uint(a.pos_over_neg);
  if (xq < a.qpr) {
    const int x4 = xq * 4;
    const float cz = ctrz[a.z_global0 + zl];
    float zt[3];
#pragma unroll
    for (int q = 0; q < 3; ++q) zt[q] = ORDER == TSDF_XFORM_PCL_SSE ? cz * a.m[4 * q + 2] + a.m[4 * q + 3] : a.m[4 * q + 2] * cz;
    const unsigned voff = (unsigned)(ty * (int)a.pitch + x4) * 4u;
    const unsigned row_step = (unsigned)a.TY * (unsigned)a.pitch * 4u;

    auto issue = [&](const int r, PipeRow &R) {
      const f4 ytv = s_yt[ty + r * a.TY];
      asm volatile("" ::: "memory");
      int pix[4];
      project_quad_allin<ORDER>(a, a.m, cam, s_cx[tid], ytv, zt, pix, R.gz);
      const unsigned soff = (unsigned)r * row_step;
      const bool d_read = !(r < 64 && (quiet >> r & 1ull));
      if (d_read)
        R.d4 = bload128(rsD, voff, soff);
      else
        asm volatile("" : "=v"(R.d4));
      R.k4 = bload32(rsK, voff >> 2, soff >> 2);
#pragma unroll
      for (int j = 0; j < 4; ++j) R.z[j] = tsdf_struct_buffer_load_u32(rsFi, pix[j], 0, 0, TSDF_GATHER_AUX);
      if (COUNT) rdb += (d_read ? 16u : 0u) + 4u;
    };

    auto consume = [&](const int r, const PipeRow &R) {
// ... 815 lines not shown
  const float a = fabsf(v);
  return nextafterf(a, INFINITY) - a;
}

struct IntegrateHost {
  IntegrateArgs a;
  float band_u, band_v;
  double fx, fy;
  int planes;
};

static IntegrateHost make_args(tsdf_handle h, const float T[12]) {
  const tsdf_params &p = h->p;
  IntegrateHost hh;
  IntegrateArgs &a = hh.a;
  for (int i = 0; i < 12; ++i) a.m[i] = T[i];
  hh.fx = p.fx;
  hh.fy = p.fy;
  a.fxf = (float)p.fx;
  a.fyf = (float)p.fy;
  {
    auto band = [](double c, int n) {
      const double q = std::max(fabs(c) + 1.0, fabs((double)n + 1.0 - c));
      const double e = q * (2.0 / 16777216.0 + 1.0 / 4194304.0) * 1.0000005 + ((double)n + 2.0) / 16777216.0 +
                       2.0 * f32_ulp((float)c) + 1e-9;
      return nextafterf((float)(1.5 * e), INFINITY);
    };
    hh.band_u = band(p.cx, p.image_width);
    hh.band_v = band(p.cy, p.image_height);
    a.cxf = (float)(p.cx + (double)hh.band_u);
    a.cyf = (float)(p.cy + (double)hh.band_v);
    a.hb_u = nextafterf(2.f * hh.band_u, INFINITY);
    a.hb_v = nextafterf(2.f * hh.band_v, INFINITY);
    a.hb_max = std::max(a.hb_u, a.hb_v);
  }
  a.zmin = p.min_sensor_dist;
  a.zlo = p.min_sensor_dist > 0.f ? nextafterf(p.min_sensor_dist, -INFINITY) : 0.f;
  a.zmax = p.max_sensor_dist;
  a.pos = p.max_dist_pos;
  a.neg = p.max_dist_neg;
  a.wmax = p.max_weight;
  a.kmax = h->kmax;
  a.kcap = h->kmax ? (h->kmax - 1u) << 24 : 0u;
  a.kinc = h->kmax ? 0x01000000u : 0u;
  a.wmax_is_int = p.max_weight == floorf(p.max_weight);
  a.pos_over_neg = p.max_dist_pos / p.max_dist_neg;
  {
    const volatile float pv = a.pos_over_neg;
    bool fixed = h->packed && a.wmax_is_int && std::isnormal(a.pos_over_neg);
    for (unsigned k = 0; fixed && k <= h->kmax; ++k) {
      const volatile float w = fminf((float)k, p.max_weight);
      const volatile float num = pv * w;
      const volatile float sum = num + pv;
      const volatile float den = w + 1.f;
      const volatile float q = sum / den;
      fixed = q == pv;
    }
    a.hinge_fixed = fixed ? 1 : 0;
  }
  a.neg_in_window = p.max_dist_neg >= 0x1p-20f && p.max_dist_neg <= 0x1p20f && p.max_dist_pos <= 0x1p20f;
  a.W = p.image_width;
  a.H = p.image_height;
  a.ny = h->ny;
  a.plane_rows = h->ny;
  a.qpr = (h->nx + 3) / 4;
  hh.planes = h->z_end - h->z_begin;
  a.z_global0 = h->z_begin;
  a.zl0 = h->z_begin - h->z_first;
  int l2 = 0;
  while ((1 << l2) < a.qpr && l2 < 8) ++l2;
  a.log2TX = l2;
  a.TX = 1 << l2;
  a.TY = 256 / a.TX;
  a.rpb = std::max(1, std::min(tsdf_tuning().rows_per_block, 256) / a.TY);
  a.rpb = std::max(1, std::min(a.rpb, (a.ny + a.TY - 1) / a.TY));
  a.pitch = h->pitch;
  a.expf_fused_r = h->expf_fused_r;
  a.ref_cull = h->ref_cull ? 1 : 0;
  for (int i = 0; i < 24; ++i) a.cull[i] = h->ref_cull ? h->cull_planes[i] : 0.f;
  a.band_fx = h->band_fx;
  a.band_fy = h->band_fy;
  a.x_abs0 = a.y_abs0 = 0;
  a.zfast = 0;
  return hh;
}

template <int ORDER>
static __global__ void __launch_bounds__(256)
k_integrate_rgbn(const IntegrateArgs a, float *__restrict__ D, float *__restrict__ Wt, uint32_t *__restrict__ RGB,
                 float *__restrict__ RN, float *__restrict__ GN, float *__restrict__ BN, float *__restrict__ IN,
                 const float *__restrict__ depth, const uint32_t *__restrict__ bgra, const double *__restrict__ cam,
                 const float *__restrict__ ctrx, const float *__restrict__ ctry, const float *__restrict__ ctrz,
                 unsigned long long *__restrict__ n_obs) {
  const int x = (int)(blockIdx.x * 256u + threadIdx.x);
  const int y = (int)blockIdx.y, zl = (int)blockIdx.z;
  bool observed = false;
  if (x < (int)a.pitch) {
    const float cx = ctrx[x], cy = ctry[y], cz = ctrz[a.z_global0 + zl];
    float g[3];
#pragma unroll
    for (int q = 0; q < 3; ++q)
      g[q] = ORDER == TSDF_XFORM_PCL_SSE ? cx * a.m[4 * q] + (cy * a.m[4 * q + 1] + (cz * a.m[4 * q + 2] + a.m[4 * q + 3]))
                                         : ((a.m[4 * q] * cx + a.m[4 * q + 1] * cy) + a.m[4 * q + 2] * cz) + a.m[4 * q + 3];
    const bool in = !(g[2] < a.zmin || g[2] > a.zmax) && g[2] > 0.f &&
                    (!a.ref_cull || reference_cull_keeps(a, cx, cy, cz));
    const int pix = in ? project_exact(a, cam, g[0], g[1], g[2]) : -1;
    if (pix >= 0) {
      const float z = depth[pix];
      float dn = z - g[2];
      if (!isnan(z) && !(dn < -a.neg)) {
        dn = dn > a.pos ? a.pos_over_neg : dn / a.neg;
        const int64_t vi = ((int64_t)(a.zl0 + zl) * a.plane_rows + y) * a.pitch + x;
        const uint32_t c = bgra[pix];
        const float r = (float)((c >> 16) & 255u), gch = (float)((c >> 8) & 255u), b = (float)(c & 255u);
        float w = Wt[vi], d = D[vi];
        const float wn = 1.f;
        const float wsum = w + wn;
        const float i = sqrtf(r * r + gch * gch + b * b);
        const float rf = r / i, gf = gch / i, bf = b / i;
        const float rn = (w * RN[vi] + wn * rf) / wsum;
        const float gn = (w * GN[vi] + wn * gf) / wsum;
        const float bn = (w * BN[vi] + wn * bf) / wsum;
        const float im = (w * IN[vi] + wn * i) / wsum;
        RN[vi] = rn;
        GN[vi] = gn;
        BN[vi] = bn;
        IN[vi] = im;
        RGB[vi] = ((uint32_t)(int)(rn * im) & 255u) | (((uint32_t)(int)(gn * im) & 255u) << 8) |
                  (((uint32_t)(int)(bn * im) & 255u) << 16);
        uint32_t unused = 0;
        add_observation_ieee<false>(d, w, unused, dn, 0u, a.wmax);
        D[vi] = d;
        Wt[vi] = w;
        observed = true;
      }
    }
  }
  if (n_obs) {
    const unsigned long long m = __ballot(observed);
    if ((threadIdx.x & 63u) == 0u && m)
      atomicAdd(n_obs + ((blockIdx.x + blockIdx.y * gridDim.x + blockIdx.z * gridDim.x * gridDim.y) & 1023u),
                (unsigned long long)__popcll(m));
  }
}

static __device__ __forceinline__ float lab_f(float t) {
  return (double)t > 0.008856 ? (float)pow((double)t, 1 / 3.) : (float)(7.787 * (double)t + (16 / 116.));
}

static __global__ void __launch_bounds__(256)
k_lab_image(const uint32_t *__restrict__ bgra, const float *__restrict__ lut, float4 *__restrict__ lab, int n) {
  const int i = (int)(blockIdx.x * 256u + threadIdx.x);
  if (i >= n) return;
  const uint32_t c = bgra[i];
  const double rf = (double)lut[(c >> 16) & 255u], gf = (double)lut[(c >> 8) & 255u], bf = (double)lut[c & 255u];
  float X = (float)(rf * 0.4124 + gf * 0.3576 + bf * 0.1805);
  float Y = (float)(rf * 0.2126 + gf * 0.7152 + bf * 0.0722);
  float Z = (float)(rf * 0.0193 + gf * 0.1192 + bf * 0.9505);
  X = (float)((double)X / 95.047);
  Y = (float)((double)Y / 100.);
  Z = (float)((double)Z / 108.883);
  X = lab_f(X);
  Y = lab_f(Y);
  Z = lab_f(Z);
  lab[i] = make_float4((116.f * Y) - 16.f, 500.f * (X - Y), 200.f * (Y - Z), 0.f);
}
// ... 225 lines not shown
    for (int r = 0; r < 3; ++r) {
      const double c = inv[3 * r] * (g[0] - t[0]) + inv[3 * r + 1] * (g[1] - t[1]) + inv[3 * r + 2] * (g[2] - t[2]);
      if (!std::isfinite(c)) return false;
      mn[r] = std::min(mn[r], c);
      mx[r] = std::max(mx[r], c);
      big = std::max(big, fabs(c));
    }
  }
  for (int a = 0; a < 3; ++a) {
    const std::vector<float> &ctr = h->h_ctr[a];
    const int n = (int)ctr.size();
    const double margin = 2.0 * (double)p.size[a] / (double)p.res[a] + 1e-5 * (big + fabs((double)p.size[a]));
    if (mx[a] + margin < (double)ctr.front() || mn[a] - margin > (double)ctr.back()) *empty = true;
    lo[a] = (int)(std::lower_bound(ctr.begin(), ctr.end(), (float)(mn[a] - margin)) - ctr.begin());
    hi[a] = (int)(std::upper_bound(ctr.begin(), ctr.end(), (float)(mx[a] + margin)) - ctr.begin()) - 1;
    if (lo[a] > 0) --lo[a];
    if (hi[a] < n - 1) ++hi[a];
    if (lo[a] > hi[a]) *empty = true;
  }
  return true;
}

static bool zlo_margin_ok(const float T[12], const tsdf_hip_volume *h) {
  double big = 0, zmin = 1e300;
  for (int k = 0; k < 8; ++k) {
    const double x = h->h_ctr[0][(k & 1) ? h->nx - 1 : 0], y = h->h_ctr[1][(k & 2) ? h->ny - 1 : 0],
                 z = h->h_ctr[2][(k & 4) ? h->z_end - 1 : h->z_begin];
    for (int r = 0; r < 3; ++r) {
      const double g = fabs((double)T[4 * r] * x) + fabs((double)T[4 * r + 1] * y) + fabs((double)T[4 * r + 2] * z) + fabs((double)T[4 * r + 3]);
      big = std::max(big, g);
    }
    zmin = std::min(zmin, (double)T[8] * x + (double)T[9] * y + (double)T[10] * z + (double)T[11]);
  }
  const double err = 8.0 * 6e-8 * big;
  const double f = std::max(fabs(h->p.fx), fabs(h->p.fy));
  return err < 1e-4 && zmin > 0.05 && f * err * (1.0 + big / zmin) / zmin < 0.05;
}

static bool reference_cull_keeps_whole_slab(const tsdf_hip_volume *h, const float *planes) {
  for (int k = 0; k < 6; ++k) {
    const float *pl = planes + 4 * k;
    double worst = -1e300, mag = 0;
    for (int c = 0; c < 8; ++c) {
      const double x = h->h_ctr[0][(c & 1) ? h->nx - 1 : 0], y = h->h_ctr[1][(c & 2) ? h->ny - 1 : 0],
                   z = h->h_ctr[2][(c & 4) ? h->z_end - 1 : h->z_begin];
      const double v = (double)pl[0] * x + (double)pl[1] * y + (double)pl[2] * z + (double)pl[3];
      if (!std::isfinite(v)) return false;
      worst = std::max(worst, v);
      mag = std::max(mag, fabs((double)pl[0] * x) + fabs((double)pl[1] * y) + fabs((double)pl[2] * z) + fabs((double)pl[3]));
    }
    if (!(worst + 8.0 * 4.0 * 5.97e-8 * mag <= 0.0)) return false;
  }
  return true;
}

static bool row_intervals_usable(const tsdf_hip_volume *h, bool planes) {
  if (h->pitch > 0xfff0 || !h->ctr_increasing[0]) return false;
  if (planes)
    for (int i = 0; i < 24; ++i)
      if (!(fabsf(h->cull_planes[i]) < 1e30f)) return false;
  return true;
}

static bool slab_all_inside(const tsdf_hip_volume *h, const float T[12]) {
  const tsdf_params &p = h->p;
  bool all_inside = true;
  for (int k = 0; k < 8 && all_inside; ++k) {
    const double x = h->h_ctr[0][(k & 1) ? h->nx - 1 : 0], y = h->h_ctr[1][(k & 2) ? h->ny - 1 : 0],
                 z = h->h_ctr[2][(k & 4) ? h->z_end - 1 : h->z_begin];
    double g[3];
    for (int r = 0; r < 3; ++r) g[r] = (double)T[4 * r] * x + (double)T[4 * r + 1] * y + (double)T[4 * r + 2] * z + (double)T[4 * r + 3];
    const double u = p.fx * g[0] / g[2] + p.cx, v = p.fy * g[1] / g[2] + p.cy;
    const double zlo = p.min_sensor_dist > 0 ? p.min_sensor_dist : 0;
    all_inside = g[2] > zlo + 1e-3 && g[2] > 1e-3 && g[2] < p.max_sensor_dist - 1e-3 && u > 1 && u < p.image_width - 2 && v > 1 &&
                 v < p.image_height - 2;
  }
  return all_inside;
}

int tsdf_integrate_launch(tsdf_handle h, const float *d_depth, const uint32_t *d_bgra, const float T[12], bool count) {
  const tsdf_params &p = h->p;
  h->count_slots = 0;
  h->count_ran = false;
  const IntegrateHost hh = make_args(h, T);
  IntegrateArgs a = hh.a;
  unsigned gx = (unsigned)((a.qpr + a.TX - 1) / a.TX);
  unsigned gy = (unsigned)((a.ny + a.rpb * a.TY - 1) / (a.rpb * a.TY));
  unsigned gz = (unsigned)hh.planes;
  if (gy > 65535u || gz > 65535u) {
    tsdf_set_error("grid too large for one launch");
    return TSDF_HIP_E_UNSUPPORTED;
  }
  const bool color = p.integrate_color != 0;
  if (color && !d_bgra) {
    tsdf_set_error("integrate_color is set but no colour image was given");
    return TSDF_HIP_E_INVALID;
  }
  if (h->weight_by_variance && (!h->vm || !h->vn || h->packed || h->cn[0])) {
    tsdf_set_error("weight_by_variance_ (hpp:203-204) needs the per-voxel M_ / nsample_ planes: F32W layout, TSDF_COLOR_RGB");
    return TSDF_HIP_E_UNSUPPORTED;
  }
  const bool rc = h->ref_cull && !reference_cull_keeps_whole_slab(h, h->cull_planes);
  const bool rc_rows = rc && !h->cn[0] && !tsdf_tuning().refcull_plain && row_intervals_usable(h, true);
  const int plain_mode = h->weight_by_depth ? 2 : h->weight_by_variance ? 4 : (rc && !rc_rows && !h->cn[0]) ? 3 : (tsdf_tuning().plain_kernel && !h->packed && !h->cn[0] ? 1 : 0);
  a.ref_cull = rc ? 1 : 0;
  if (plain_mode || h->cn[0]) h->band_exact = false;
  if (plain_mode) {
    if ((h->packed && plain_mode != 3) || h->cn[0]) {
      tsdf_set_error("weight_by_depth needs the F32W layout and TSDF_COLOR_RGB");
      return TSDF_HIP_E_UNSUPPORTED;
    }
    if (count) TSDF_HIP_TRY(hipMemsetAsync(h->counter, 0, 1024 * sizeof(unsigned long long), h->stream));
    bool pose_ok = true;
    for (int i = 0; i < 12; ++i) pose_ok &= std::isfinite(T[i]) && fabsf(T[i]) <= 1e15f;
    if (pose_ok) {
      const dim3 grid((unsigned)((h->pitch + 255) / 256), (unsigned)h->ny, gz), block(256);
      if (grid.y > 65535u) {
        tsdf_set_error("grid too large for one launch");
        return TSDF_HIP_E_UNSUPPORTED;
      }
#define LAUNCH_PLAIN(ORDER, COLOR, BYD, PK)                                                                             \
  hipLaunchKernelGGL((k_integrate_plain<ORDER, COLOR, BYD, PK>), grid, block, 0, h->stream, a, h->d, h->w, h->rgb, h->k8, \
                     h->weight_by_variance ? h->vm : nullptr, h->weight_by_variance ? h->vn : nullptr, d_depth, d_bgra,   \
                     h->cam64, h->ctr[0], h->ctr[1], h->ctr[2], count ? h->counter : nullptr)
#define LP2(ORDER, COLOR)                      \
  do {                                         \
    if (plain_mode == 2)                       \
      LAUNCH_PLAIN(ORDER, COLOR, true, false); \
    else if (h->packed)                        \
      LAUNCH_PLAIN(ORDER, COLOR, false, true); \
    else                                       \
      LAUNCH_PLAIN(ORDER, COLOR, false, false); \
  } while (0)
      if (p.xform_order == TSDF_XFORM_PCL_SSE) {
        if (color)
          LP2(TSDF_XFORM_PCL_SSE, true);
        else
          LP2(TSDF_XFORM_PCL_SSE, false);
      } else {
        if (color)
          LP2(TSDF_XFORM_LEFT_TO_RIGHT, true);
        else
          LP2(TSDF_XFORM_LEFT_TO_RIGHT, false);
      }
#undef LP2
#undef LAUNCH_PLAIN
      TSDF_HIP_TRY(hipGetLastError());
    }
    h->count_slots = count ? 1024 : 0;
    h->count_ran = pose_ok;
    return TSDF_HIP_OK;
  }
  if (h->cn[0]) {
    if (count) TSDF_HIP_TRY(hipMemsetAsync(h->counter, 0, 1024 * sizeof(unsigned long long), h->stream));
    bool pose_ok = true;
    for (int i = 0; i < 12; ++i) pose_ok &= std::isfinite(T[i]) && fabsf(T[i]) <= 1e15f;
    if (pose_ok) {
      const dim3 grid((unsigned)((h->pitch + 255) / 256), (unsigned)h->ny, gz), block(256);
      if (grid.y > 65535u) {
        tsdf_set_error("grid too large for one launch");
        return TSDF_HIP_E_UNSUPPORTED;
      }
      if (h->lab_img) {
        const int npx = p.image_width * p.image_height;
        hipLaunchKernelGGL(k_lab_image, dim3((unsigned)((npx + 255) / 256)), dim3(256), 0, h->stream, d_bgra,
                           h->lab_lut, h->lab_img, npx);
// ... 57 lines not shown
      a.rpb = std::max(1, std::min(2 * tsdf_tuning().rows_per_block, 64) / a.TY);
      gx = (unsigned)((a.qpr + a.TX - 1) / a.TX);
      gy = (unsigned)((a.ny + a.rpb * a.TY - 1) / (a.rpb * a.TY));
    }
    int lo[3], hi[3];
    bool empty = false;
    if (tsdf_tuning().cull && !all_inside && observable_index_box(h, T, lo, hi, &empty)) {
      lo[2] = std::max(lo[2], h->z_begin);
      hi[2] = std::min(hi[2], h->z_end - 1);
      if (empty || lo[2] > hi[2]) {
        nothing_observable = true;
      } else {
        const int bxv = a.TX * 4, byr = a.rpb * a.TY;
        const int bx0 = lo[0] / bxv, bx1 = hi[0] / bxv, by0 = lo[1] / byr, by1 = hi[1] / byr;
        const int x_off = bx0 * bxv, y_off = by0 * byr, z_off = lo[2] - h->z_begin;
        const int64_t e_off = (int64_t)y_off * h->pitch + x_off;
        D += e_off;
        if (Wt) Wt += e_off;
        if (RGB) RGB += e_off;
        if (K8) K8 += e_off;
        ctrx += x_off;
        ctry += y_off;
        a.qpr -= x_off / 4;
        a.ny -= y_off;
        a.x_abs0 = x_off;
        a.y_abs0 = y_off;
        a.z_global0 += z_off;
        a.zl0 += z_off;
        gx = (unsigned)(bx1 - bx0 + 1);
        gy = (unsigned)(by1 - by0 + 1);
        gz = (unsigned)(hi[2] - lo[2] + 1);
      }
    }
    if (gy > 65535u) {
      tsdf_set_error("grid too large for one launch");
      return TSDF_HIP_E_UNSUPPORTED;
    }
    if (!nothing_observable) {
      CullArgs c;
      for (int i = 0; i < 12; ++i) c.m[i] = T[i];
      c.fx = p.fx, c.fy = p.fy, c.cx = p.cx, c.cy = p.cy;
      c.zlo = p.min_sensor_dist > 0 ? p.min_sensor_dist : 0;
      c.zmax = p.max_sensor_dist;
      c.W = p.image_width, c.H = p.image_height;
      c.nx = h->nx - (int)(ctrx - h->ctr[0]), c.ny = a.ny, c.z_global0 = a.z_global0;
      c.bx_vox = a.TX * 4, c.by_rows = a.rpb * a.TY;
      c.gx = (int)gx, c.gy = (int)gy, c.gz = (int)gz;
      const int rows = std::min(a.ny, (int)gy * a.rpb * a.TY);
      a.ny = rows;
      c.ny = rows;
      RowArgs ra;
      for (int i = 0; i < 12; ++i) ra.m[i] = T[i];
      ra.fx = p.fx, ra.fy = p.fy, ra.cx = p.cx, ra.cy = p.cy;
      ra.zlo = c.zlo, ra.zmax = c.zmax;
      ra.W = c.W, ra.H = c.H;
      ra.nx = std::min(c.nx, (int)gx * a.TX * 4), ra.ny = rows, ra.nz = (int)gz, ra.z_global0 = a.z_global0;
      ra.rc = rc_rows ? 1 : 0;
      for (int i = 0; i < 24; ++i) ra.cull[i] = rc_rows ? h->cull_planes[i] : 0.f;
      const size_t nb = (size_t)gx * gy * gz, nrows = (size_t)rows * gz;
      if (nb > h->live_cap || nrows > h->row_iv_cap) {
        TSDF_HIP_TRY(hipStreamSynchronize(h->stream));
        if (nb > h->live_cap) {
          if (h->live) TSDF_HIP_TRY(hipFree(h->live));
          h->live = nullptr, h->live_cap = 0;
          TSDF_HIP_TRY(hipMalloc(&h->live, nb));
          h->live_cap = nb;
        }
        if (nrows > h->row_iv_cap) {
          if (h->row_iv) TSDF_HIP_TRY(hipFree(h->row_iv));
          h->row_iv = nullptr, h->row_iv_cap = 0;
          TSDF_HIP_TRY(hipMalloc(&h->row_iv, nrows * sizeof(uint32_t)));
          h->row_iv_cap = nrows;
        }
      }
      if (ra.nx <= TSDF_ROWS_LDS_NX)
        hipLaunchKernelGGL(k_rows<true>, dim3((unsigned)((nrows + 255) / 256)), dim3(256), 0, h->stream, ra, ctrx, ctry, h->ctr[2], h->row_iv);
      else
        hipLaunchKernelGGL(k_rows<false>, dim3((unsigned)((nrows + 255) / 256)), dim3(256), 0, h->stream, ra, ctrx, ctry, h->ctr[2], h->row_iv);
      hipLaunchKernelGGL(k_cull, dim3((unsigned)((nb + 255) / 256)), dim3(256), 0, h->stream, c, ctrx, ctry, h->ctr[2], h->row_iv, h->live);
      TSDF_HIP_TRY(hipGetLastError());
      live = h->live;
    }
  }
  if (count) TSDF_HIP_TRY(hipMemsetAsync(h->counter, 0, 4096 * sizeof(unsigned long long), h->stream));
  bool pose_ok = true;
  for (int i = 0; i < 12; ++i) pose_ok &= std::isfinite(T[i]) && fabsf(T[i]) <= 1e15f;
  const bool fastproj = fast_projection_ok(hh, p.integrate_color != 0);
  h->last_launch[0] = h->last_launch[1] = h->last_launch[2] = h->last_launch[3] = 0;
  uint8_t *band_arg = h->band_exact && ((a.rpb * a.TY) & 3) == 0 && (a.y_abs0 & 3) == 0 ? h->band : nullptr;
  if (!band_arg) h->band_exact = false;
  a.implied_d = implied_distances(h, a, band_arg != nullptr);
  h->last_implied_on = a.implied_d != 0;
  if (pose_ok && !nothing_observable) {
    const size_t frame_bytes = npx * (color ? 8 : 4);
    a.zfast = tsdf_tuning().zfast < 0 ? (frame_bytes > (3u << 20) && gx <= 65535u) : (tsdf_tuning().zfast != 0 && gx <= 65535u);
    const dim3 grid(a.zfast ? gz : gx, gy, a.zfast ? gx : gz), block(256);
    h->last_launch[0] = fastproj && allin && !live;
    h->last_launch[1] = fastproj;
    h->last_launch[2] = live ? (rc_rows ? 2 : 1) : 0;
    h->last_launch[3] = (int)std::min<uint64_t>((uint64_t)gx * gy * gz, 0x7fffffffu);
#define LAUNCH(ORDER, COLOR, FP, COUNT, PK, AI, LV)                                                                  \
  hipLaunchKernelGGL((k_integrate<ORDER, COLOR, FP, COUNT, PK, AI, LV>), grid, block, 0, h->stream, a, D, Wt, RGB, K8, \
                     d_depth, h->cam64, ctrx, ctry, h->ctr[2], h->counter, live, band_arg, h->row_iv)
#define L6(ORDER, COLOR, FP, COUNT, PK)                  \
  do {                                                   \
    if (live)                                            \
      LAUNCH(ORDER, COLOR, FP, COUNT, PK, false, true);  \
    else if (FP && allin)                                \
      LAUNCH(ORDER, COLOR, FP, COUNT, PK, FP, false);    \
    else                                                 \
      LAUNCH(ORDER, COLOR, FP, COUNT, PK, false, false); \
  } while (0)
#define L5(ORDER, COLOR, FP, COUNT)     \
  do {                                  \
    if (h->packed)                      \
      L6(ORDER, COLOR, FP, COUNT, true);  \
    else                                \
      L6(ORDER, COLOR, FP, COUNT, false); \
  } while (0)
#define L4(ORDER, COLOR, FP) \
  do {                       \
    if (count)               \
      L5(ORDER, COLOR, FP, true);  \
    else                     \
      L5(ORDER, COLOR, FP, false); \
  } while (0)
#define L2(ORDER, COLOR) \
  do {                   \
    if (fastproj)        \
      L4(ORDER, COLOR, true);  \
    else                 \
      L4(ORDER, COLOR, false); \
  } while (0)
    const bool pipe = (tsdf_tuning().pipe & (color ? 2 : 1)) && fastproj && allin && !live && h->packed && a.hinge_fixed && a.neg_in_window &&
                      a.ny % a.TY == 0;
    if (pipe) {
      h->last_launch[0] |= 0x100;
#define LAUNCH_P(ORDER, COUNT)                                                                                                           \
  do {                                                                                                                                   \
    if (color)                                                                                                                           \
      hipLaunchKernelGGL((k_integrate_pc<ORDER, COUNT>), grid, block, 0, h->stream, a, D, RGB, d_depth, h->cam64, ctrx, ctry, h->ctr[2], \
                         h->counter, band_arg);                                                                                          \
    else                                                                                                                                 \
      hipLaunchKernelGGL((k_integrate_p<ORDER, COUNT>), grid, block, 0, h->stream, a, D, K8, d_depth, h->cam64, ctrx, ctry, h->ctr[2],   \
                         h->counter, band_arg);                                                                                          \
  } while (0)
      if (p.xform_order == TSDF_XFORM_PCL_SSE) {
        if (count)
          LAUNCH_P(TSDF_XFORM_PCL_SSE, true);
        else
          LAUNCH_P(TSDF_XFORM_PCL_SSE, false);
      } else {
        if (count)
          LAUNCH_P(TSDF_XFORM_LEFT_TO_RIGHT, true);
        else
          LAUNCH_P(TSDF_XFORM_LEFT_TO_RIGHT, false);
      }
#undef LAUNCH_P
    } else if (p.xform_order == TSDF_XFORM_PCL_SSE) {
      if (color)
        L2(TSDF_XFORM_PCL_SSE, true);
      else
        L2(TSDF_XFORM_PCL_SSE, false);
    } else {
      if (color)
        L2(TSDF_XFORM_LEFT_TO_RIGHT, true);
      else
        L2(TSDF_XFORM_LEFT_TO_RIGHT, false);
    }
#undef L2
#undef L4
#undef L5
#undef L6
#undef LAUNCH
    TSDF_HIP_TRY(hipGetLastError());
#if TSDF_PHASE_TIMER
    if (const char *pf = getenv("TSDF_HIP_PHASE_FILE")) {
      TSDF_HIP_TRY(hipStreamSynchronize(h->stream));
      static unsigned long long host_ph[1024 * TSDF_NPHASE];
      TSDF_HIP_TRY(hipMemcpyFromSymbol(host_ph, HIP_SYMBOL(g_phase), sizeof host_ph));
      unsigned long long sum[TSDF_NPHASE] = {0};
      for (int i = 0; i < 1024; ++i)
        for (int k = 0; k < TSDF_NPHASE; ++k) sum[k] += host_ph[i * TSDF_NPHASE + k];
      memset(host_ph, 0, sizeof host_ph);
      TSDF_HIP_TRY(hipMemcpyToSymbol(HIP_SYMBOL(g_phase), host_ph, sizeof host_ph));
      if (FILE *f = fopen(pf, "a")) {
        fprintf(f, "{\"color\": %d, \"count\": %d, \"allin\": %d, \"live\": %d, \"packed\": %d, \"blocks\": %d, \"phase\": [", (int)color, (int)count,
                (int)(fastproj && allin && !live), (int)(live != nullptr), (int)h->packed, h->last_launch[3]);
        for (int k = 0; k < TSDF_NPHASE; ++k) fprintf(f, "%llu%s", sum[k], k + 1 < TSDF_NPHASE ? ", " : "]}\n");
        fclose(f);
      }
    }
#endif
  }
  h->count_slots = count ? 4096 : 0;
  h->count_ran = pose_ok && !nothing_observable;
  return TSDF_HIP_OK;
}

int tsdf_integrate_collect(tsdf_handle h, uint64_t *n_observed) {
  if (!h->count_slots) {
    tsdf_set_error("tsdf_integrate_collect without a counting launch");
    return TSDF_HIP_E_INVALID;
  }
  unsigned long long c[4096];
  const int slots = h->count_slots;
  TSDF_HIP_TRY(hipMemcpyAsync(c, h->counter, (size_t)slots * sizeof(unsigned long long), hipMemcpyDeviceToHost, h->stream));
  TSDF_HIP_TRY(hipStreamSynchronize(h->stream));
  unsigned long long sum = 0, changed = 0, implied = 0, read_bytes = 0;
  for (int i = 0; i < 1024; ++i) sum += c[i];
  for (int i = 1024; i < slots && i < 2048; ++i) changed += c[i];
  for (int i = 2048; i < slots && i < 3072; ++i) implied += c[i];
  for (int i = 3072; i < slots; ++i) read_bytes += c[i];
  h->last_observed = h->count_ran ? sum : 0;
  h->last_changed_bytes = h->count_ran ? changed : 0;
  h->last_implied = h->count_ran ? implied : 0;
  h->last_read_bytes = h->count_ran ? read_bytes : 0;
  h->count_slots = 0;
  if (n_observed) *n_observed = h->last_observed;
  return TSDF_HIP_OK;
}

static int launch_integrate(tsdf_handle h, const float *d_depth, const uint32_t *d_bgra, const float T[12],
                            uint64_t *n_observed) {
  const int rc = tsdf_integrate_launch(h, d_depth, d_bgra, T, n_observed != nullptr);
  if (rc || !n_observed) return rc;
  return tsdf_integrate_collect(h, n_observed);
}

static bool fusable_pose(tsdf_handle h, const IntegrateHost &hh, const float T[12], const float *planes) {
  for (int i = 0; i < 12; ++i)
    if (!(std::isfinite(T[i]) && fabsf(T[i]) <= 1e15f)) return false;
  if (planes && !reference_cull_keeps_whole_slab(h, planes)) return false;
  return slab_all_inside(h, T) && zlo_margin_ok(T, h) && fast_projection_ok(hh, h->p.integrate_color != 0);
}

int tsdf_integrate_launch2(tsdf_handle h, const float *dA, const uint32_t *cA, const float TA[12], const float *planesA_,
                           const float *dB, const uint32_t *cB, const float TB[12], const float *planesB_, bool count, bool *fused) {
  float planes_copy[2][24];
  const float *planesA = nullptr, *planesB = nullptr;
  if (planesA_) memcpy(planes_copy[0], planesA_, sizeof planes_copy[0]), planesA = planes_copy[0];
  if (planesB_) memcpy(planes_copy[1], planesB_, sizeof planes_copy[1]), planesB = planes_copy[1];
  const tsdf_params &p = h->p;
  const bool color = p.integrate_color != 0;
  if (color && (!cA || !cB)) {
    tsdf_set_error("integrate_color is set but no colour image was given");
    return TSDF_HIP_E_INVALID;
  }
  const IntegrateHost hh = make_args(h, TA);
  IntegrateArgs a = hh.a;
  const size_t npx = (size_t)p.image_width * p.image_height;
  auto bgra_offset = [&](const float *d, const uint32_t *c, unsigned *off) {
    *off = 0;
    if (!color) return true;
    const char *zd = (const char *)d, *cb = (const char *)c;
    if (!(cb >= zd + npx * 4 && (size_t)(cb - zd) + npx * 4 < (1ull << 31))) return false;
    *off = (unsigned)(cb - zd);
    return true;
  };
  Frame2 fb;
  for (int i = 0; i < 12; ++i) fb.m[i] = TB[i];
  const unsigned gx = (unsigned)((a.qpr + a.TX - 1) / a.TX), gy = (unsigned)((a.ny + a.rpb * a.TY - 1) / (a.rpb * a.TY)),
                 gz = (unsigned)hh.planes;
  const bool pipe_wins = !color && (tsdf_tuning().pipe & 1) && tsdf_tuning().fuse2 == 1 && a.hinge_fixed && a.neg_in_window && a.ny % a.TY == 0;
  const bool ok = tsdf_tuning().fuse2 && !pipe_wins && tsdf_tuning().cull == 1 && tsdf_tuning().allin && h->packed && !h->cn[0] && !h->weight_by_depth &&
                  !h->weight_by_variance && !tsdf_tuning().plain_kernel && (h->nx & 3) == 0 && a.wmax_is_int && (float)h->kmax == p.max_weight &&
                  gy <= 65535u && gz <= 65535u && gz > 0 && bgra_offset(dA, cA, &a.bgra_off) && bgra_offset(dB, cB, &fb.bgra_off) &&
                  fusable_pose(h, hh, TA, planesA) && fusable_pose(h, hh, TB, planesB);
  if (fused) *fused = ok;
  if (!ok) {
    int rc = tsdf_hip_set_reference_cull(h, planesA);
    if (!rc) rc = tsdf_integrate_launch(h, dA, cA, TA, count);
    if (!rc && count) {
      uint64_t n = 0;
      rc = tsdf_integrate_collect(h, &n);
      h->pair_first_observed = n, h->pair_first_changed = h->last_changed_bytes, h->pair_first_implied = h->last_implied;
      h->pair_first_read = h->last_read_bytes;
    }
    if (!rc) rc = tsdf_hip_set_reference_cull(h, planesB);
    if (!rc) rc = tsdf_integrate_launch(h, dB, cB, TB, count);
    h->pair_fused = false;
    return rc;
  }
  h->ref_cull = planesB != nullptr;
  for (int i = 0; i < 24; ++i) h->cull_planes[i] = planesB ? planesB[i] : 0.f;
  h->count_slots = 0;
  h->count_ran = false;
  if (count) TSDF_HIP_TRY(hipMemsetAsync(h->counter, 0, 3072 * sizeof(unsigned long long), h->stream));
  uint8_t *band_arg = h->band_exact && ((a.rpb * a.TY) & 3) == 0 ? h->band : nullptr;
  if (!band_arg) h->band_exact = false;
  (void)implied_distances(h, a, band_arg != nullptr);
  a.implied_d = 0;
  h->last_implied_on = false;
  h->last_launch[0] = 2, h->last_launch[1] = 1, h->last_launch[2] = 0;
  h->last_launch[3] = (int)std::min<uint64_t>((uint64_t)gx * gy * gz, 0x7fffffffu);
  a.zfast = tsdf_tuning().zfast < 0 ? (npx * (color ? 8 : 4) > (3u << 20) && gx <= 65535u) : (tsdf_tuning().zfast != 0 && gx <= 65535u);
  const dim3 grid(a.zfast ? gz : gx, gy, a.zfast ? gx : gz), block(256);
#define LAUNCH2(ORDER, COLOR, COUNT)                                                                                    \
  hipLaunchKernelGGL((k_integrate2<ORDER, COLOR, COUNT>), grid, block, 0, h->stream, a, fb, h->d, h->rgb, h->k8, dA, dB, \
                     h->cam64, h->ctr[0], h->ctr[1], h->ctr[2], h->counter, band_arg)
#define L2B(ORDER, COLOR)         \
// ... 7 lines not shown
    if (color)
      L2B(TSDF_XFORM_PCL_SSE, true);
    else
      L2B(TSDF_XFORM_PCL_SSE, false);
  } else {
    if (color)
      L2B(TSDF_XFORM_LEFT_TO_RIGHT, true);
    else
      L2B(TSDF_XFORM_LEFT_TO_RIGHT, false);
  }
#undef L2B
#undef LAUNCH2
  TSDF_HIP_TRY(hipGetLastError());
  h->count_slots = count ? 3072 : 0;
  h->count_ran = true;
  h->pair_fused = true;
  return TSDF_HIP_OK;
}

int tsdf_integrate_collect2(tsdf_handle h, uint64_t n_observed[2]) {
  if (!h->pair_fused) {
    uint64_t nb = 0;
    const int rc = tsdf_integrate_collect(h, &nb);
    if (rc) return rc;
    n_observed[0] = h->pair_first_observed, n_observed[1] = nb;
    h->last_observed = h->pair_first_observed + nb;
    h->last_changed_bytes += h->pair_first_changed;
    h->last_implied += h->pair_first_implied;
    h->last_read_bytes += h->pair_first_read;
    return TSDF_HIP_OK;
  }
  if (!h->count_slots) {
    tsdf_set_error("tsdf_integrate_collect2 without a counting launch");
    return TSDF_HIP_E_INVALID;
  }
  unsigned long long c[3072];
  TSDF_HIP_TRY(hipMemcpyAsync(c, h->counter, sizeof c, hipMemcpyDeviceToHost, h->stream));
  TSDF_HIP_TRY(hipStreamSynchronize(h->stream));
  unsigned long long sum[6] = {0, 0, 0, 0, 0, 0};
  for (int i = 0; i < 3072; ++i) sum[i >> 9] += c[i];
  n_observed[0] = sum[0], n_observed[1] = sum[1];
  h->last_observed = sum[2];
  h->last_changed_bytes = sum[3];
  h->last_implied = sum[4];
  h->last_read_bytes = sum[5];
  h->count_slots = 0;
  return TSDF_HIP_OK;
}

extern "C" int tsdf_hip_integrate_device2(tsdf_handle h, const float *d_depth_a, const uint32_t *d_bgra_a, const float cam_from_vol_a[12],
                                          const float *planes_a, const float *d_depth_b, const uint32_t *d_bgra_b,
                                          const float cam_from_vol_b[12], const float *planes_b, uint64_t *n_observed, int32_t *fused) {
  if (!h || !d_depth_a || !d_depth_b || !cam_from_vol_a || !cam_from_vol_b) return TSDF_HIP_E_INVALID;
  if (fused) *fused = 0;
  if (h->multi)
    return tsdf_multi_integrate_device2(h, d_depth_a, d_bgra_a, cam_from_vol_a, planes_a, d_depth_b, d_bgra_b, cam_from_vol_b, planes_b,
                                        n_observed, fused);
  TSDF_ENTER(h);
  bool f = false;
  const int rc = tsdf_integrate_launch2(h, d_depth_a, d_bgra_a, cam_from_vol_a, planes_a, d_depth_b, d_bgra_b, cam_from_vol_b, planes_b,
                                        n_observed != nullptr, &f);
  if (fused) *fused = f ? 1 : 0;
  if (rc || !n_observed) return rc;
  return tsdf_integrate_collect2(h, n_observed);
}

extern "C" int tsdf_hip_last_count_detail(tsdf_handle h, uint64_t out[2]) {
  if (!h || !out) return TSDF_HIP_E_INVALID;
  if (h->multi) return tsdf_multi_last_count_detail(h, out);
  out[0] = h->last_observed;
  out[1] = h->last_changed_bytes;
  return TSDF_HIP_OK;
}

extern "C" int tsdf_hip_last_read_detail(tsdf_handle h, uint64_t out[3]) {
  if (!h || !out) return TSDF_HIP_E_INVALID;
  if (h->multi) return tsdf_multi_last_read_detail(h, out);
  out[0] = h->last_implied;
  out[1] = h->last_implied_on ? 1 : 0;
  out[2] = h->last_read_bytes;
  return TSDF_HIP_OK;
}

extern "C" int tsdf_hip_set_reference_cull(tsdf_handle h, const float planes[24]) {
  if (!h) return TSDF_HIP_E_INVALID;
  if (h->multi) return tsdf_multi_set_reference_cull(h, planes);
  h->ref_cull = planes != nullptr;
  for (int i = 0; i < 24; ++i) h->cull_planes[i] = planes ? planes[i] : 0.f;
  return TSDF_HIP_OK;
}

extern "C" int tsdf_hip_last_launch_info(tsdf_handle h, int32_t out[4]) {
  if (!h || !out) return TSDF_HIP_E_INVALID;
  if (h->multi) h = tsdf_multi_first(h);
  for (int i = 0; i < 4; ++i) out[i] = h->last_launch[i];
  return TSDF_HIP_OK;
}

static int host_expf_fuses_r() {
  volatile float probe = -0x1.f8cbb2p+5f;
  return expf(probe) == 0x1.f45326p-92f ? 1 : 0;
}

static __global__ void k_expf(const float *__restrict__ in, float *__restrict__ out, size_t n, int fused_r) {
  const size_t i = (size_t)blockIdx.x * blockDim.x + threadIdx.x;
  if (i < n) out[i] = tsdf_expf_glibc(in[i], fused_r != 0);
}
static int device_expf(const float *in, size_t n, float *out, int fused_r) {
  float *di = nullptr, *dout = nullptr;
  TSDF_HIP_TRY(hipMalloc(&di, n * 4));
  TSDF_HIP_TRY(hipMalloc(&dout, n * 4));
  TSDF_HIP_TRY(hipMemcpy(di, in, n * 4, hipMemcpyHostToDevice));
  hipLaunchKernelGGL(k_expf, dim3((unsigned)((n + 255) / 256)), dim3(256), 0, 0, di, dout, n, fused_r);
  TSDF_HIP_TRY(hipGetLastError());
  TSDF_HIP_TRY(hipMemcpy(out, dout, n * 4, hipMemcpyDeviceToHost));
  (void)hipFree(di);
  (void)hipFree(dout);
  return TSDF_HIP_OK;
}

static int expf_matches_this_host(int fused_r) {
  static int verdict = -1;
  if (verdict >= 0) return verdict;
  const size_t n = 4096;
  std::vector<float> in(n), dev(n);
  uint32_t s = 0x9e3779b9u;
  for (size_t i = 0; i < n; ++i) {
    s = s * 1664525u + 1013904223u;
    const float u = (float)(s >> 8) * (1.0f / 16777216.0f);
    const float mag = ldexpf(1.0f + u, (int)(i % 34) - 26);
    in[i] = (i & 1) ? mag : -mag;
  }
  if (device_expf(in.data(), n, dev.data(), fused_r) != TSDF_HIP_OK) return -1;
  verdict = 1;
  for (size_t i = 0; i < n; ++i) {
    const volatile float x = in[i];
    const float want = expf(x);
    if (memcmp(&want, &dev[i], 4) != 0 && !(std::isnan(want) && std::isnan(dev[i]))) verdict = 0;
  }
  return verdict;
}

extern "C" int tsdf_hip_set_weighting(tsdf_handle h, int weight_by_depth, int weight_by_variance) {
  if (!h) return TSDF_HIP_E_INVALID;
  if (h->multi) return tsdf_multi_set_weighting(h, weight_by_depth, weight_by_variance);
  if (weight_by_depth && (h->packed || h->cn[0])) {
    tsdf_set_error("weight_by_depth makes weights non-integer: it needs the F32W layout (and TSDF_COLOR_RGB)");
    return TSDF_HIP_E_UNSUPPORTED;
  }
  if (weight_by_variance && (h->packed || h->cn[0])) {
    tsdf_set_error("weight_by_variance needs float weights and TSDF_COLOR_RGB: create / load the volume with TSDF_LAYOUT_F32W");
    return TSDF_HIP_E_UNSUPPORTED;
  }
  TSDF_ENTER(h);
  if (weight_by_variance && !h->vm) {
    const size_t n = (size_t)(h->pitch * h->ny * h->nz_alloc);
    TSDF_HIP_TRY(hipMalloc(&h->vm, n * sizeof(float)));
    TSDF_HIP_TRY(hipMalloc(&h->vn, n * sizeof(int32_t)));
    TSDF_HIP_TRY(hipMemsetAsync(h->vm, 0, n * sizeof(float), h->stream));
    TSDF_HIP_TRY(hipMemsetAsync(h->vn, 0, n * sizeof(int32_t), h->stream));
  }
  h->expf_fused_r = host_expf_fuses_r();
  if (weight_by_variance) {
    TSDF_ON_DEVICE(h->device);
    if (expf_matches_this_host(h->expf_fused_r) == 0) {
      tsdf_set_error("weight_by_variance_: this host's expf is not the glibc algorithm the device restates (4096-float spot check "
// ... 620 lines not shown
```

### cpu_tsdf_amd/csrc/tsdf_multi.hip

```cpp
#include <string.h>

#include <algorithm>
#include <thread>
#include <vector>

#include "tsdf_common.h"
#include "tsdf_occupied.h"
#include "tsdf_flatten.h"
#include "tsdf_meshpost.h"

struct tsdf_hip_multi {
  std::vector<tsdf_handle> slab;
  std::vector<hipStream_t> stream;
  int halo = 0;
  float *pinned[2] = {nullptr, nullptr};
  std::vector<hipEvent_t> uploaded[2];
  unsigned long long frames = 0;
  bool pairing = false;
  std::vector<hipEvent_t> ev, ev2;
  bool halo1_fresh = false, halo_all_fresh = false;
  int frame_staged = 0;
  std::vector<int *> ray_list, ray_outbox, ray_finbox;
  std::vector<unsigned *> ray_counters;
  int *ray_fin_in = nullptr;
// ... 555 lines not shown
  tsdf_hip_multi *m = h->multi;
  const size_t npx = (size_t)h->p.image_width * h->p.image_height;
  const bool color = h->p.integrate_color != 0;
  if (color && !d_bgra) {
    tsdf_set_error("integrate_color is set but no colour image was given");
    return TSDF_HIP_E_INVALID;
  }
  int src_dev = -1;
  {
    hipPointerAttribute_t attr;
    if (hipPointerGetAttributes(&attr, d_depth) == hipSuccess)
      src_dev = attr.device;
    else
      (void)hipGetLastError();
  }
  if (src_dev < 0) {
    tsdf_set_error("d_depth is not a device pointer");
    return TSDF_HIP_E_INVALID;
  }
  if (src_slab >= 0) {
    TSDF_ON_DEVICE(m->slab[src_slab]->device);
    TSDF_HIP_TRY(hipEventRecord(m->ev[src_slab], m->slab[src_slab]->stream));
  }
  for (size_t k = 0; k < m->slab.size(); ++k) {
    tsdf_handle s = m->slab[k];
    if ((int)k == src_slab) continue;
    TSDF_ON_DEVICE(s->device);
    if (src_slab >= 0) TSDF_HIP_TRY(hipStreamWaitEvent(s->stream, m->ev[src_slab], 0));
    if (d_depth != s->frame_depth) {
      const int rc = tsdf_multi_copy(m, s->frame_depth, s->device, d_depth, src_dev, npx * 4, s->stream);
      if (rc) return rc;
    }
    if (color && d_bgra != s->frame_bgra) {
      const int rc = tsdf_multi_copy(m, s->frame_bgra, s->device, d_bgra, src_dev, npx * 4, s->stream);
      if (rc) return rc;
    }
    if (src_slab >= 0) TSDF_HIP_TRY(hipEventRecord(m->ev2[k], s->stream));
  }
  if (src_slab >= 0) {
    TSDF_ON_DEVICE(m->slab[src_slab]->device);
    for (size_t k = 0; k < m->slab.size(); ++k)
      if ((int)k != src_slab) TSDF_HIP_TRY(hipStreamWaitEvent(m->slab[src_slab]->stream, m->ev2[k], 0));
  }
  return TSDF_HIP_OK;
}

int tsdf_multi_integrate_device(tsdf_handle h, const float *d_depth, const uint32_t *d_bgra, const float T[12],
                                uint64_t *n_observed) {
  if (const int rc_flush = tsdf_multi_flush(h)) return rc_flush;
  int rc = fan_out_device(h, d_depth, d_bgra, -1);
  if (rc) return rc;
  return integrate_all(h, T, n_observed);
}

int tsdf_multi_organize(tsdf_handle h, const float *xyz, size_t xyz_stride, const uint8_t *bgra, size_t bgra_stride, size_t n,
                        float cloud_units, int zero_nans, const double world_to_cam[12], float *depth_out, uint8_t *bgra_out,
                        uint64_t *n_valid) {
  const int rc = tsdf_hip_organize(h->multi->slab[0], xyz, xyz_stride, bgra, bgra_stride, n, cloud_units, zero_nans, world_to_cam,
                                   depth_out, bgra_out, n_valid);
  if (!rc) h->multi->frame_staged = 1;
  return rc;
}

int tsdf_multi_integrate_staged(tsdf_handle h, const float T[12], uint64_t *n_observed) {
  if (const int rc_flush = tsdf_multi_flush(h)) return rc_flush;
  tsdf_hip_multi *m = h->multi;
  if (!m->frame_staged) {
    tsdf_set_error("no staged frame: call tsdf_hip_organize first");
    return TSDF_HIP_E_INVALID;
  }
  tsdf_handle s0 = m->slab[0];
  int rc = fan_out_device(h, s0->frame_depth, s0->p.integrate_color ? s0->frame_bgra : nullptr, 0);
  if (rc) return rc;
  return integrate_all(h, T, n_observed);
}

int tsdf_multi_last_read_detail(tsdf_handle h, uint64_t out[3]) {
  out[0] = h->last_implied;
  out[1] = h->last_implied_on ? 1 : 0;
  out[2] = h->last_read_bytes;
  return TSDF_HIP_OK;
}

int tsdf_multi_last_count_detail(tsdf_handle h, uint64_t out[2]) {
  out[0] = h->last_observed;
  out[1] = h->last_changed_bytes;
  return TSDF_HIP_OK;
}

static int copy_planes(tsdf_hip_multi *m, int src, int dst, int z0, int nz) {
  tsdf_handle a = m->slab[src], b = m->slab[dst];
  const int64_t plane = a->pitch * a->ny;
  const int64_t oa = (int64_t)(z0 - a->z_first) * plane, ob = (int64_t)(z0 - b->z_first) * plane;
  {
    TSDF_ON_DEVICE(a->device);
    TSDF_HIP_TRY(hipEventRecord(m->ev[src], a->stream));
  }
  TSDF_ON_DEVICE(b->device);
  TSDF_HIP_TRY(hipStreamWaitEvent(b->stream, m->ev[src], 0));
  auto cp = [&](void *dst_p, const void *src_p, size_t bytes) -> int {
    return tsdf_multi_copy(m, dst_p, b->device, src_p, a->device, bytes, b->stream);
  };
  const size_t n = (size_t)(plane * nz);
  int rc = cp(b->d + ob, a->d + oa, n * 4);
  if (!rc && a->w) rc = cp(b->w + ob, a->w + oa, n * 4);
  if (!rc && a->rgb) rc = cp(b->rgb + ob, a->rgb + oa, n * 4);
  if (!rc && a->k8) rc = cp(b->k8 + ob, a->k8 + oa, n);
  for (int c = 0; c < 4 && !rc; ++c)
    if (a->cn[c]) rc = cp(b->cn[c] + ob, a->cn[c] + oa, n * 4);
  return rc;
}

static int all_wait_all(tsdf_hip_multi *m) {
  const int n = (int)m->slab.size();
  for (int k = 0; k < n; ++k) {
    TSDF_ON_DEVICE(m->slab[k]->device);
    TSDF_HIP_TRY(hipEventRecord(m->ev2[k], m->slab[k]->stream));
  }
  for (int k = 0; k < n; ++k) {
    TSDF_ON_DEVICE(m->slab[k]->device);
    for (int j = 0; j < n; ++j)
      if (j != k) TSDF_HIP_TRY(hipStreamWaitEvent(m->slab[k]->stream, m->ev2[j], 0));
  }
  return TSDF_HIP_OK;
}

static int exchange_halo(tsdf_handle h, int planes, bool both) {
  tsdf_hip_multi *m = h->multi;
  const int n = (int)m->slab.size();
  if (n == 1) return TSDF_HIP_OK;
  planes = std::min(planes, m->halo);
  if (both ? m->halo_all_fresh : (m->halo1_fresh && planes <= 1)) return TSDF_HIP_OK;
  for (int k = 0; k < n; ++k) {
    tsdf_handle s = m->slab[k];
    const int ranges[2][2] = {{s->z_end, std::min(h->nz, s->z_end + planes)},
                              {both ? std::max(0, s->z_begin - planes) : s->z_begin, s->z_begin}};
    for (int r = 0; r < 2; ++r)
      for (int z = ranges[r][0]; z < ranges[r][1];) {
        const int o = owner_of(m, z);
        if (o < 0) return TSDF_HIP_E_INVALID;
        const int run = std::min(ranges[r][1], m->slab[o]->z_end) - z;
        const int rc = copy_planes(m, o, k, z, run);
        if (rc) return rc;
        z += run;
      }
  }
  if (int rc = all_wait_all(m)) return rc;
  m->halo1_fresh = true;
  if (both && planes >= m->halo) m->halo_all_fresh = true;
  return TSDF_HIP_OK;
}

int tsdf_multi_block(tsdf_handle h, bool down, int x0, int y0, int z0, int nx, int ny, int nz, float *d, float *w, uint8_t *rgb) {
  if (const int rc_flush = tsdf_multi_flush(h)) return rc_flush;
  tsdf_hip_multi *m = h->multi;
  if (nx <= 0 || ny <= 0 || nz <= 0 || z0 < 0 || z0 + nz > h->nz) {
    tsdf_set_error("block outside the grid");
    return TSDF_HIP_E_INVALID;
  }
  if (!down) m->halo1_fresh = m->halo_all_fresh = false;
  const size_t per_plane = (size_t)nx * ny;
  for (int z = z0; z < z0 + nz;) {
    const int o = owner_of(m, z);
    const int run = std::min(z0 + nz, m->slab[o]->z_end) - z;
    const size_t off = (size_t)(z - z0) * per_plane;
    const int rc = down ? tsdf_hip_download(m->slab[o], x0, y0, z, nx, ny, run, d ? d + off : nullptr, w ? w + off : nullptr,
// ... 391 lines not shown
```

### include/tsdf_hip.h

```cpp
#ifndef TSDF_HIP_H
#define TSDF_HIP_H

#include <stddef.h>
#include <stdint.h>

#ifdef __cplusplus
extern "C" {
#endif

typedef struct tsdf_hip_volume *tsdf_handle;

enum {
  TSDF_HIP_OK = 0,
  TSDF_HIP_E_INVALID = 1,
  TSDF_HIP_E_NOMEM = 2,
  TSDF_HIP_E_HIP = 3,
  TSDF_HIP_E_NODEVICE = 4,
  TSDF_HIP_E_UNSUPPORTED = 5,
  TSDF_HIP_E_IO = 6,
  TSDF_HIP_ALIGN_NO_POINTS = 7,
  TSDF_HIP_ALIGN_RANK_DEFICIENT = 8
};

enum {
  TSDF_XFORM_PCL_SSE = 0,
  TSDF_XFORM_LEFT_TO_RIGHT = 1
};

enum { TSDF_LAYOUT_AUTO = 0, TSDF_LAYOUT_F32W = 1, TSDF_LAYOUT_PACKED = 2 };

enum {
  TSDF_COLOR_RGB = 0,
  TSDF_COLOR_RGB_NORMALIZED = 1,
  TSDF_COLOR_LAB = 2
};

typedef struct tsdf_params {
  int32_t res[3];
  float size[3];
  float max_dist_pos;
  float max_dist_neg;
  float max_weight;
  float min_sensor_dist;
  float max_sensor_dist;
  double fx, fy, cx, cy;
  int32_t image_width;
  int32_t image_height;
  int32_t integrate_color;
  int32_t xform_order;
  int32_t z_begin, z_end;
  int32_t halo;
  int32_t device;
  int32_t layout;
  int32_t color_mode;
} tsdf_params;

void tsdf_hip_default_params(tsdf_params *p);

int tsdf_hip_create(const tsdf_params *p, tsdf_handle *out);
int tsdf_hip_reset(tsdf_handle h);
int tsdf_hip_destroy(tsdf_handle h);

int tsdf_hip_create_multi(const tsdf_params *p, const int32_t *devices, int n_devices, tsdf_handle *out);
int tsdf_hip_slab_count(tsdf_handle h);
int tsdf_hip_multi_render_stats(tsdf_handle h, uint64_t out[4]);
int tsdf_hip_multi_link_stats(tsdf_handle h, uint64_t out[3]);
int tsdf_hip_multi_timing(tsdf_handle h, int enable);
int tsdf_hip_multi_kernel_ms(tsdf_handle h, int k, float *ms_sum, int32_t *launches);
int tsdf_hip_slab_info(tsdf_handle h, int k, int32_t *device, int32_t *z_begin, int32_t *z_end, int32_t *halo);

int tsdf_hip_host_alloc(size_t bytes, void **out);
int tsdf_hip_host_free(void *p);

int tsdf_hip_set_stream(tsdf_handle h, void *hip_stream);
int tsdf_hip_synchronize(tsdf_handle h);

int tsdf_hip_integrate(tsdf_handle h, const float *depth, const uint8_t *bgra,
                       const float cam_from_vol[12], uint64_t *n_observed);
int tsdf_hip_integrate_device(tsdf_handle h, const float *d_depth, const uint32_t *d_bgra,
                              const float cam_from_vol[12], uint64_t *n_observed);
int tsdf_hip_integrate_async(tsdf_handle h, const float *depth, const uint8_t *bgra,
                             const float cam_from_vol[12]);
int tsdf_hip_frame_begin(tsdf_handle h, float **depth, uint8_t **bgra);
int tsdf_hip_frame_commit(tsdf_handle h, const float cam_from_vol[12]);

int tsdf_hip_organize(tsdf_handle h, const float *xyz, size_t xyz_stride, const uint8_t *bgra,
                      size_t bgra_stride, size_t n, float cloud_units, int zero_nans,
                      const double world_to_cam[12], float *depth_out, uint8_t *bgra_out, uint64_t *n_valid);
int tsdf_hip_integrate_staged(tsdf_handle h, const float cam_from_vol[12], uint64_t *n_observed);

int tsdf_hip_last_count_detail(tsdf_handle h, uint64_t out[2]);
int tsdf_hip_last_read_detail(tsdf_handle h, uint64_t out[3]);

int tsdf_hip_set_weighting(tsdf_handle h, int weight_by_depth, int weight_by_variance);

int tsdf_hip_download_variance_state(tsdf_handle h, int x0, int y0, int z0, int nx, int ny, int nz, float *M, int32_t *nsample);
int tsdf_hip_upload_variance_state(tsdf_handle h, int x0, int y0, int z0, int nx, int ny, int nz, const float *M,
                                   const int32_t *nsample);

int tsdf_hip_raycast(tsdf_handle h, const float rot[9], const float origin[3], int downsample,
                     float *out);
int tsdf_hip_raycast_camera(tsdf_handle h, const float rot[9], const float origin[3], int downsample,
                            const double cam_from_vol[12], float *out);

#define TSDF_HIP_RAY_RECORD_INTS 24
int tsdf_hip_raycast_begin(tsdf_handle h, const float rot[9], const float origin[3], int downsample,
                           int32_t *d_state);
int tsdf_hip_raycast_advance(tsdf_handle h, const float rot[9], const float origin[3], int downsample,
                             int rank, int world, const int32_t *d_state, int32_t *d_delta);
int tsdf_hip_raycast_advance_list(tsdf_handle h, const float rot[9], const float origin[3], int downsample,
                                  int rank, int world, int32_t *d_records, size_t count);
int tsdf_hip_render_halo(const tsdf_params *p);

int tsdf_hip_alloc_probe(tsdf_handle h, float ms[8], int32_t *chosen);

int tsdf_hip_set_reference_cull(tsdf_handle h, const float planes[24]);
int tsdf_hip_integrate_device2(tsdf_handle h, const float *d_depth_a, const uint32_t *d_bgra_a, const float cam_from_vol_a[12],
                               const float *planes_a, const float *d_depth_b, const uint32_t *d_bgra_b,
                               const float cam_from_vol_b[12], const float *planes_b, uint64_t *n_observed, int32_t *fused);

int tsdf_hip_set_frame_pairing(tsdf_handle h, int on);

int tsdf_hip_reference_cull_planes(const tsdf_params *p, const double trans[16], float planes[24]);
int tsdf_hip_reference_cull_is_noop(const tsdf_params *p);

int tsdf_hip_sample(tsdf_handle h, const float *xyz, size_t n, float *val, float *grad,
                    float *hess, uint8_t *ok);

int tsdf_hip_lookup_rgb(tsdf_handle h, const float *xyz, size_t n, uint8_t *rgb, uint8_t *found);

int tsdf_hip_align_system(tsdf_handle h, const float *xyz, size_t n, const double vol_from_src[12],
                          float min_weight, float r_max, double out[29], uint8_t *used, float *xyz_vol);
int tsdf_hip_align_system_device(tsdf_handle h, const float *d_xyz, size_t n, const double vol_from_src[12],
                                 float min_weight, float r_max, double out[29]);
int tsdf_hip_align(tsdf_handle h, const float *xyz, size_t n, const double guess[12], float min_weight, float r_max,
                   int max_iterations, double min_step, double refined[12], int32_t *iterations, double *cost_log);
int tsdf_hip_align_stats(tsdf_handle h, uint64_t out[4]);

int tsdf_hip_march(tsdf_handle h, float w_min, int color_mode, uint64_t *n_tri);
int tsdf_hip_march_fetch(tsdf_handle h, float *verts, uint8_t *rgb, uint64_t *cell);
int tsdf_hip_march_timing(tsdf_handle h, float ms[3], uint64_t *n_cells);
int tsdf_hip_march_stats(tsdf_handle h, uint64_t out[4]);
int tsdf_hip_march_fetch_device(tsdf_handle h, float *d_verts, uint8_t *d_rgb, uint64_t *d_cell);

int tsdf_hip_mesh_cleanup(int device, const float *verts, uint64_t n_verts, const uint32_t *faces ,
                          uint64_t n_faces, float face_dist, int min_neighbors, uint8_t *keep, uint64_t *n_kept);
int tsdf_hip_march_cleanup(tsdf_handle h, float face_dist, int min_neighbors, uint64_t *n_tri);
int tsdf_hip_mesh_cleanup_stats(uint64_t out[4]);

int tsdf_hip_mesh_flatten(int device, const float *verts, uint64_t n_verts, const uint32_t *faces ,
                          uint64_t n_faces, float min_dist, uint32_t *remap, uint32_t *seeds, uint64_t *n_out_verts,
                          uint32_t *out_faces, uint64_t *n_out_faces);
int tsdf_hip_march_flatten(tsdf_handle h, float min_dist, uint64_t *n_verts, uint64_t *n_faces);
int tsdf_hip_march_fetch_indexed(tsdf_handle h, float *verts, uint8_t *rgb, uint32_t *faces, uint64_t *cell);
int tsdf_hip_mesh_flatten_stats(uint64_t out[4]);

int tsdf_hip_occupied(tsdf_handle h, const int32_t box[6], uint64_t *n);
int tsdf_hip_occupied_fetch(tsdf_handle h, int32_t *idx, float *d, float *w, uint8_t *rgb);
int tsdf_hip_occupied_fetch_device(tsdf_handle h, int32_t *d_idx, float *d_d, float *d_w, uint32_t *d_rgb);
int tsdf_hip_occupied_stats(tsdf_handle h, uint64_t out[4]);
int tsdf_hip_occupied_timing(tsdf_handle h, float ms[3]);

int tsdf_hip_download(tsdf_handle h, int x0, int y0, int z0, int nx, int ny, int nz, float *d,
                      float *w, uint8_t *rgb);
int tsdf_hip_upload(tsdf_handle h, int x0, int y0, int z0, int nx, int ny, int nz, const float *d,
                    const float *w, const uint8_t *rgb);

int tsdf_hip_download_color_state(tsdf_handle h, int plane_index, int z0, int nz, float *out);

typedef struct tsdf_vol_meta {
  float max_cell_size[3];
  int32_t is_empty;
  int32_t weight_by_depth;
  int32_t weight_by_variance;
  double global_transform[16];
// ... 38 lines not shown
```

Measured before the change: 666,800.

## Classify voxel row segments against per-frame depth-tile min/max bounds to skip or shortcut work

A new kernel builds a per-frame table of 8x8 depth tile min/max values with a sparse-table hierarchy per tile row. The integrate kernel projects each 64-voxel row segment's endpoints, queries the covered tiles, and marks the segment hidden (behind all surface plus truncation, so it is skipped) or free (fully in front, so depth gathers are skipped and the voxel is updated with the positive truncation value). Blocks whose rows are all hidden exit early. This adds an extra kernel launch, shared-memory traffic and a row-class readfirstlane per row. The path is only used when the pipelined kernel is not selected, and it brings diagnostic counters plus a query API.

```diff
diff --git a/cpu_tsdf_amd/capi.py b/cpu_tsdf_amd/capi.py
--- a/cpu_tsdf_amd/capi.py
+++ b/cpu_tsdf_amd/capi.py
@@ -98,6 +98,7 @@
     "tsdf_hip_frame_commit": (C.c_int, [C.c_void_p, _f32p]),
     "tsdf_hip_last_count_detail": (C.c_int, [C.c_void_p, _u64p]),
     "tsdf_hip_last_read_detail": (C.c_int, [C.c_void_p, _u64p]),
+    "tsdf_hip_last_row_classes": (C.c_int, [C.c_void_p, _u64p]),
     "tsdf_hip_march_timing": (C.c_int, [C.c_void_p, _f32p, _u64p]),
     "tsdf_hip_march_stats": (C.c_int, [C.c_void_p, _u64p]),
     "tsdf_hip_raycast": (C.c_int, [C.c_void_p, _f32p, _f32p, C.c_int, _f32p]),
diff --git a/cpu_tsdf_amd/csrc/tsdf_common.h b/cpu_tsdf_amd/csrc/tsdf_common.h
--- a/cpu_tsdf_amd/csrc/tsdf_common.h
+++ b/cpu_tsdf_amd/csrc/tsdf_common.h
@@ -10,6 +10,7 @@
 
 struct tsdf_hip_pipeline;
 struct tsdf_hip_multi;
+struct TsdfDB2;
 
 struct tsdf_hip_volume {
   tsdf_hip_multi *multi = nullptr;
@@ -57,6 +58,10 @@
   size_t live_cap = 0;
   uint32_t *row_iv = nullptr;
   size_t row_iv_cap = 0;
+  TsdfDB2 *db_tab = nullptr;
+  size_t db_cap = 0;
+  int db_mode_counted = 0;
+  unsigned long long last_row_classes[5] = {0, 0, 0, 0, 0};
   bool ctr_increasing[3] = {false, false, false};
   unsigned long long *counter = nullptr;
   unsigned long long last_observed = 0, last_changed_bytes = 0;
@@ -106,6 +111,7 @@
 int tsdf_multi_integrate_staged(tsdf_handle h, const float T[12], uint64_t *n_observed);
 int tsdf_multi_last_count_detail(tsdf_handle h, uint64_t out[2]);
 int tsdf_multi_last_read_detail(tsdf_handle h, uint64_t out[3]);
+int tsdf_multi_last_row_classes(tsdf_handle h, uint64_t out[5]);
 int tsdf_multi_block(tsdf_handle h, bool down, int x0, int y0, int z0, int nx, int ny, int nz, float *d, float *w, uint8_t *rgb);
 int tsdf_multi_sample(tsdf_handle h, const float *xyz, size_t n, float *val, float *grad, float *hess, uint8_t *ok);
 int tsdf_multi_align_system(tsdf_handle h, const float *xyz, size_t n, const double vol_from_src[12], float min_weight, float r_max,
@@ -251,6 +257,7 @@
   int implied_d;
   int pipe;
   int lab_chunk;
+  int depth_bounds;
 };
 const TsdfTuning &tsdf_tuning();
 int tsdf_vol_chunk();
@@ -296,6 +303,110 @@
   return v.rgb[i] & 0xffffffu;
 }
 
+#define TSDF_DB_TILE_LOG2 3
+#define TSDF_DB_MAX_TW 1024
+struct __attribute__((aligned(8))) TsdfDB2 {
+  float mx, mn;
+};
+struct TsdfDepthBounds {
+  const TsdfDB2 *tab;
+  int W, H;
+  int tw, th;
+  int levels;
+};
+enum { TSDF_ROW_GENERAL = 0, TSDF_ROW_HIDDEN = 1, TSDF_ROW_FREE = 2 };
+
+static inline __host__ __device__ int tsdf_db_levels(int tw) {
+  int l = 1;
+  while ((1 << l) <= tw) ++l;
+  return l;
+}
+static inline __host__ __device__ size_t tsdf_db_entries(int W, int H) {
+  const int tw = (W + 7) >> TSDF_DB_TILE_LOG2, th = (H + 7) >> TSDF_DB_TILE_LOG2;
+  return (size_t)th * (size_t)tsdf_db_levels(tw) * (size_t)tw;
+}
+static inline __host__ __device__ TsdfDB2 tsdf_db_tile(const float *depth, int W, int H, int tx, int ty) {
+  const float inf = __builtin_inff();
+  TsdfDB2 e = {-inf, inf};
+  bool nan = false;
+  const int x0 = tx << TSDF_DB_TILE_LOG2, y0 = ty << TSDF_DB_TILE_LOG2;
+  for (int y = y0; y < y0 + 8 && y < H; ++y)
+    for (int x = x0; x < x0 + 8 && x < W; ++x) {
+      const float z = depth[(size_t)y * (size_t)W + (size_t)x];
+      if (z != z) {
+        nan = true;
+      } else {
+        e.mx = z > e.mx ? z : e.mx;
+        e.mn = z < e.mn ? z : e.mn;
+      }
+    }
+  if (nan) e.mn = -inf;
+  return e;
+}
+static inline __host__ __device__ TsdfDB2 tsdf_db_combine(const TsdfDB2 a, const TsdfDB2 b) {
+  TsdfDB2 e;
+  e.mx = a.mx > b.mx ? a.mx : b.mx;
+  e.mn = a.mn < b.mn ? a.mn : b.mn;
+  return e;
+}
+static inline void tsdf_db_build_host(const float *depth, int W, int H, TsdfDB2 *tab) {
+  const int tw = (W + 7) >> TSDF_DB_TILE_LOG2, th = (H + 7) >> TSDF_DB_TILE_LOG2, levels = tsdf_db_levels(tw);
+  for (int ty = 0; ty < th; ++ty) {
+    TsdfDB2 *row = tab + (size_t)ty * levels * tw;
+    for (int t = 0; t < tw; ++t) row[t] = tsdf_db_tile(depth, W, H, t, ty);
+    for (int k = 1; k < levels; ++k)
+      for (int t = 0; t < tw; ++t) {
+        const int u = t + (1 << (k - 1));
+        row[(size_t)k * tw + t] = u < tw ? tsdf_db_combine(row[(size_t)(k - 1) * tw + t], row[(size_t)(k - 1) * tw + u]) : row[(size_t)(k - 1) * tw + t];
+      }
+  }
+}
+static inline __host__ __device__ TsdfDB2 tsdf_db_query(const TsdfDepthBounds &b, int t0, int t1, int r0, int r1) {
+  int k = 0;
+  while ((2 << k) <= t1 - t0 + 1) ++k;
+  const float inf = __builtin_inff();
+  TsdfDB2 e = {-inf, inf};
+  for (int r = r0; r <= r1; ++r) {
+    const TsdfDB2 *lv = b.tab + ((size_t)r * b.levels + k) * b.tw;
+    e = tsdf_db_combine(e, tsdf_db_combine(lv[t0], lv[t1 - (1 << k) + 1]));
+  }
+  return e;
+}
+
+static inline __host__ __device__ void tsdf_row_point(const float m[12], bool pcl_sse, float cx, float cy, float cz, float g[3]) {
+  for (int q = 0; q < 3; ++q) {
+    if (pcl_sse) {
+      const float yt = cy * m[4 * q + 1] + (cz * m[4 * q + 2] + m[4 * q + 3]);
+      g[q] = cx * m[4 * q] + yt;
+    } else {
+      const float yt = m[4 * q + 1] * cy, zt = m[4 * q + 2] * cz;
+      g[q] = ((cx * m[4 * q] + yt) + zt) + m[4 * q + 3];
+    }
+  }
+}
+
+static inline __host__ __device__ int tsdf_classify_segment(const float g0[3], const float g1[3], double fx, double fy, double cx, double cy,
+                                                            const TsdfDepthBounds &b, float pos, float neg, int *box = nullptr) {
+  if (box) box[0] = box[1] = box[2] = box[3] = 0;
+  if (!(g0[2] > 0.f) || !(g1[2] > 0.f)) return TSDF_ROW_GENERAL;
+  const double ua = (double)g0[0] * fx / (double)g0[2] + cx, ub = (double)g1[0] * fx / (double)g1[2] + cx;
+  const double va = (double)g0[1] * fy / (double)g0[2] + cy, vb = (double)g1[1] * fy / (double)g1[2] + cy;
+  const double ulo = ua < ub ? ua : ub, uhi = ua < ub ? ub : ua, vlo = va < vb ? va : vb, vhi = va < vb ? vb : va;
+  if (!(ulo > -1e9 && uhi < 1e9 && vlo > -1e9 && vhi < 1e9)) return TSDF_ROW_GENERAL;
+  int u0 = (int)floor(ulo) - 1, u1 = (int)floor(uhi) + 1, v0 = (int)floor(vlo) - 1, v1 = (int)floor(vhi) + 1;
+  if (u1 < 0 || v1 < 0 || u0 > b.W - 1 || v0 > b.H - 1) return TSDF_ROW_GENERAL;
+  u0 = u0 < 0 ? 0 : u0, v0 = v0 < 0 ? 0 : v0, u1 = u1 > b.W - 1 ? b.W - 1 : u1, v1 = v1 > b.H - 1 ? b.H - 1 : v1;
+  if (box) box[0] = u0, box[1] = u1, box[2] = v0, box[3] = v1;
+  const int t0 = u0 >> TSDF_DB_TILE_LOG2, t1 = u1 >> TSDF_DB_TILE_LOG2, r0 = v0 >> TSDF_DB_TILE_LOG2, r1 = v1 >> TSDF_DB_TILE_LOG2;
+  if (r1 - r0 + 1 > 4) return TSDF_ROW_GENERAL;
+  const TsdfDB2 e = tsdf_db_query(b, t0, t1, r0, r1);
+  const float gz_lo = g0[2] < g1[2] ? g0[2] : g1[2], gz_hi = g0[2] < g1[2] ? g1[2] : g0[2];
+  const float far_raw = e.mx - gz_lo, near_raw = e.mn - gz_hi;
+  if (far_raw < -neg) return TSDF_ROW_HIDDEN;
+  if (near_raw > pos && near_raw >= -neg) return TSDF_ROW_FREE;
+  return TSDF_ROW_GENERAL;
+}
+
 static inline __host__ __device__ int64_t tsdf_index(int64_t pitch, int ny, int z_first, int x, int y,
                                                       int zg) {
   return ((int64_t)(zg - z_first) * ny + y) * pitch + x;
diff --git a/cpu_tsdf_amd/csrc/tsdf_core.hip b/cpu_tsdf_amd/csrc/tsdf_core.hip
--- a/cpu_tsdf_amd/csrc/tsdf_core.hip
+++ b/cpu_tsdf_amd/csrc/tsdf_core.hip
@@ -58,7 +58,8 @@
                          env_int("TSDF_HIP_CULL", 1), std::max(1, env_int("TSDF_HIP_VOL_CHUNK", 256)),
                          env_int("TSDF_HIP_PLAIN_KERNEL", 0), env_int("TSDF_HIP_ALLOC_TRIES", 3), env_int("TSDF_HIP_ALLIN", 1),
                          env_int("TSDF_HIP_REFCULL_PLAIN", 0), env_int("TSDF_HIP_LIVE_LOG2TX", 5), env_int("TSDF_HIP_ZFAST", 1), env_int("TSDF_HIP_FUSE2", 1), env_int("TSDF_HIP_IMPLIED_D", 1),
-                         env_int("TSDF_HIP_PIPE", 1), std::max(1, env_int("TSDF_HIP_LAB_CHUNK", 16 << 20))};
+                         env_int("TSDF_HIP_PIPE", 1), std::max(1, env_int("TSDF_HIP_LAB_CHUNK", 16 << 20)),
+                         env_int("TSDF_HIP_DEPTH_BOUNDS", 1)};
   return t;
 }
 
@@ -108,6 +109,8 @@
     t.zfast = value;
   else if (n == "lab_chunk")
     t.lab_chunk = std::max(1, value);
+  else if (n == "depth_bounds")
+    t.depth_bounds = value;
   else
     return TSDF_HIP_E_INVALID;
   return TSDF_HIP_OK;
@@ -392,6 +395,7 @@
   if (v->cam64) (void)hipFree(v->cam64);
   if (v->live) (void)hipFree(v->live);
   if (v->row_iv) (void)hipFree(v->row_iv);
+  if (v->db_tab) (void)hipFree(v->db_tab);
   if (v->band) (void)hipFree(v->band);
   if (v->counter) (void)hipFree(v->counter);
   if (v->mc_verts) (void)hipFree(v->mc_verts);
@@ -652,8 +656,8 @@
   v->band_fx = (v->nx + 63) / 64;
   v->band_fy = (v->ny + 3) / 4;
   TRY_OR_BAIL(hipMalloc(&v->band, (size_t)v->band_fx * v->band_fy * v->nz_alloc));
-  TRY_OR_BAIL(hipMalloc(&v->counter, 4096 * sizeof(unsigned long long)));
-  TRY_OR_BAIL(hipMemset(v->counter, 0, 4096 * sizeof(unsigned long long)));
+  TRY_OR_BAIL(hipMalloc(&v->counter, 4104 * sizeof(unsigned long long)));
+  TRY_OR_BAIL(hipMemset(v->counter, 0, 4104 * sizeof(unsigned long long)));
 #undef TRY_OR_BAIL
   rc = tsdf_hip_reset(v);
   if (rc != TSDF_HIP_OK) return bail(rc);
diff --git a/cpu_tsdf_amd/csrc/tsdf_integrate.hip b/cpu_tsdf_amd/csrc/tsdf_integrate.hip
--- a/cpu_tsdf_amd/csrc/tsdf_integrate.hip
+++ b/cpu_tsdf_amd/csrc/tsdf_integrate.hip
@@ -50,8 +50,33 @@
   int implied_d;
   int x_abs0, y_abs0;
   int zfast;
+  int db_mode;
+  const TsdfDB2 *db_tab;
   int64_t pitch;
 };
+
+static __global__ void __launch_bounds__(256)
+k_depth_bounds(const float *__restrict__ depth, int W, int H, int tw, int levels, TsdfDB2 *__restrict__ tab) {
+  __shared__ TsdfDB2 s_lv[2][TSDF_DB_MAX_TW];
+  const int ty = (int)blockIdx.x;
+  TsdfDB2 *row = tab + (size_t)ty * (size_t)levels * (size_t)tw;
+  for (int t = (int)threadIdx.x; t < tw; t += 256) {
+    const TsdfDB2 e = tsdf_db_tile(depth, W, H, t, ty);
+    s_lv[0][t] = e;
+    row[t] = e;
+  }
+  for (int k = 1; k < levels; ++k) {
+    __syncthreads();
+    const TsdfDB2 *src = s_lv[(k - 1) & 1];
+    TsdfDB2 *dst = s_lv[k & 1];
+    for (int t = (int)threadIdx.x; t < tw; t += 256) {
+      const int u = t + (1 << (k - 1));
+      const TsdfDB2 e = u < tw ? tsdf_db_combine(src[t], src[u]) : src[t];
+      dst[t] = e;
+      row[(size_t)k * (size_t)tw + t] = e;
+    }
+  }
+}
 
 static __device__ __forceinline__ int project_exact(const IntegrateArgs &a, const double *__restrict__ cam,
                                                     float gx, float gy, float gz) {
@@ -372,6 +397,9 @@
 #define TSDF_BAND_SYNC() __syncthreads()
 #define TSDF_BAND_FIRST ((int)tid)
 #define TSDF_BAND_STEP 256
+#endif
+#ifndef TSDF_ROW_FREE_PATH
+#define TSDF_ROW_FREE_PATH 1
 #endif
 #ifndef TSDF_RECOMPUTE_PX
 #define TSDF_RECOMPUTE_PX 1
@@ -484,7 +512,9 @@
 #pragma unroll
       for (int q = 0; q < 3; ++q)
         t[q] = ORDER == TSDF_XFORM_PCL_SSE ? cy_ * a.m[4 * q + 1] + (cz_ * a.m[4 * q + 2] + a.m[4 * q + 3]) : a.m[4 * q + 1] * cy_;
-      s_yt[tid] = t;
+      float *sy = reinterpret_cast<float *>(&s_yt[tid]);
+      sy[0] = t.x, sy[1] = t.y, sy[2] = t.z;
+      if (!(ALLIN && a.db_mode && (int)tid < (256 >> (a.log2TX - 6)))) sy[3] = 0.f;
     }
     if (F2) {
       const int xq_ = (int)bc.bx * a.TX + (int)(tid & (unsigned)(a.TX - 1));
@@ -494,7 +524,42 @@
   }
   __shared__ uint8_t s_bin[PACKED ? 1024 : 1];
   if (PACKED && a.implied_d) tsdf_flags_before(a, bc, band, s_bin, tid);
+  __shared__ uint32_t s_allhid[4];
+  __shared__ uint2 s_box[COUNT && ALLIN ? 256 : 1];
+  unsigned n_rows = 0, n_hid = 0, n_fre = 0, n_viol = 0;
+  if constexpr (ALLIN) {
+    if (a.db_mode) {
+      const int lseg = a.log2TX - 6, seg = (int)tid & ((1 << lseg) - 1), rowi = (int)tid >> lseg;
+      const int yy = (int)bc.by * a.rpb * a.TY + rowi;
+      const int xq0 = (int)bc.bx * a.TX + seg * 64;
+      int cls = TSDF_ROW_HIDDEN;
+      if (rowi < a.rpb * a.TY && yy < a.ny && xq0 < a.qpr) {
+        const int xq1 = min(xq0 + 63, a.qpr - 1);
+        const float cy_ = ctry[yy], cz_ = ctrz[a.z_global0 + (int)bc.bz];
+        float g0[3], g1[3];
+        tsdf_row_point(a.m, ORDER == TSDF_XFORM_PCL_SSE, ctrx[xq0 * 4], cy_, cz_, g0);
+        tsdf_row_point(a.m, ORDER == TSDF_XFORM_PCL_SSE, ctrx[xq1 * 4 + 3], cy_, cz_, g1);
+        TsdfDepthBounds b;
+        b.tab = a.db_tab, b.W = a.W, b.H = a.H;
+        b.tw = (a.W + 7) >> TSDF_DB_TILE_LOG2, b.th = (a.H + 7) >> TSDF_DB_TILE_LOG2, b.levels = tsdf_db_levels(b.tw);
+        int box[4];
+        cls = tsdf_classify_segment(g0, g1, cam[0], cam[1], cam[2], cam[3], b, a.pos, a.neg, COUNT ? box : nullptr);
+        if (COUNT) {
+          s_box[tid] = make_uint2((unsigned)box[0] | (unsigned)box[1] << 16, (unsigned)box[2] | (unsigned)box[3] << 16);
+          n_rows = 1u, n_hid = cls == TSDF_ROW_HIDDEN ? 1u : 0u, n_fre = cls == TSDF_ROW_FREE ? 1u : 0u;
+        }
+      }
+      int nib = (a.db_mode == 1 ? cls * 5 : cls) << (4 * seg);
+      if (lseg >= 1) nib |= __shfl_xor(nib, 1);
+      if (lseg >= 2) nib |= __shfl_xor(nib, 2);
+      if (seg == 0) reinterpret_cast<uint32_t *>(&s_yt[rowi])[3] = (uint32_t)nib;
+      const uint64_t hid_m = __builtin_amdgcn_ballot_w64(cls == TSDF_ROW_HIDDEN);
+      if ((tid & 63u) == 0u) s_allhid[tid >> 6] = hid_m == ~0ull && a.rpb * a.TY <= (256 >> lseg) ? 1u : 0u;
+    }
+  }
   __syncthreads();
+  const bool use_cls = ALLIN && a.db_mode == 1;
+  if (!COUNT && use_cls && (s_allhid[0] & s_allhid[1] & s_allhid[2] & s_allhid[3])) return;
   const uint64_t quiet = PACKED && a.implied_d ? tsdf_quiet_passes(a, s_bin, tid) : 0ull;
   PT_MARK_OUT(9);
   const int tx = (int)(tid & (unsigned)(a.TX - 1));
@@ -526,6 +591,7 @@
       for (int j = 0; j < 4; ++j) px_[j][r] = cxs[j] * a.m[4 * r];
       zt[r] = ORDER == TSDF_XFORM_PCL_SSE ? cz * a.m[4 * r + 2] + a.m[4 * r + 3] : a.m[4 * r + 2] * cz;
     }
+    const unsigned cls_shift = ALLIN ? (unsigned)__builtin_amdgcn_readfirstlane((int)((tid >> 6 & (unsigned)((a.TX >> 6) - 1)) * 4u)) : 0u;
     const unsigned voff = (unsigned)(ty * (int)a.pitch + x4) * 4u;
     const unsigned row_step = (unsigned)a.TY * (unsigned)a.pitch * 4u;
 #if TSDF_EARLY_VOXEL_LOADS
@@ -541,8 +607,19 @@
         if (!((unsigned)(x4 + 3) - iv_lo < iv_len + 3u)) continue;
       }
       const unsigned soff = (unsigned)r * row_step;
-      const f4 ytv = s_yt[ty + r * a.TY];
+      int yi = ty + r * a.TY;
+      asm volatile("" : "+v"(yi));
+      const f4 ytv = s_yt[yi];
       const float yt[3] = {ytv.x, ytv.y, ytv.z};
+      unsigned rcls = 0u;
+      if (ALLIN) rcls = (unsigned)__builtin_amdgcn_readfirstlane((int)__float_as_uint(ytv.w)) >> cls_shift & 15u;
+      if (ALLIN && (rcls & 4u)) {
+#if TSDF_EARLY_VOXEL_LOADS
+        pred_obs = false;
+#endif
+        continue;
+      }
+      const bool row_free = TSDF_ROW_FREE_PATH && ALLIN && PACKED && (rcls & 8u);
 #if TSDF_RECOMPUTE_PX
       float px[4][3];
       if constexpr (!F2) {
@@ -627,7 +704,7 @@
       asm volatile("" : "=v"(d4));
       u4 w4 = {0u, 0u, 0u, 0u}, c4 = {0u, 0u, 0u, 0u};
       uint32_t k4 = 0u;
-      const bool ask_early = EARLY && (TSDF_EARLY_VOXEL_LOADS != 2 || pred_obs);
+      const bool ask_early = EARLY && (TSDF_EARLY_VOXEL_LOADS != 2 || pred_obs || row_free);
       if (ask_early) {
         if (d_read) d4 = bload128(rsD, voff, soff);
         if (COLOR) c4 = bload128(rsC, voff, soff);
@@ -643,11 +720,19 @@
           zs[j] = 1e3f + (float)(pix[j] & 1);
           cs[j] = 0x00406080u + (unsigned)pix[j];
         } else if (ALLIN) {
+          if (row_free) break;
           zs[j] = __uint_as_float(tsdf_struct_buffer_load_u32(rsFi, pix[j], 0, 0, TSDF_GATHER_AUX));
           if (COLOR) cs[j] = tsdf_struct_buffer_load_u32(rsFi, pix[j], 0, (int)a.bgra_off, TSDF_GATHER_AUX);
         } else {
           zs[j] = __uint_as_float(bload32(rsF, (unsigned)pix[j] << 2, 0u));
           if (COLOR) cs[j] = bload32(rsF, (unsigned)pix[j] << 2, a.bgra_off);
+        }
+      }
+      if (ALLIN && row_free) {
+#pragma unroll
+        for (int j = 0; j < 4; ++j) {
+          zs[j] = 0.f;
+          if (COLOR) cs[j] = tsdf_struct_buffer_load_u32(rsFi, pix[j], 0, (int)a.bgra_off, TSDF_GATHER_AUX);
         }
       }
       PT_MARK(1);
@@ -657,18 +742,41 @@
       bool act[4];
       any = false;
       bool any_div = false;
-#pragma unroll
-      for (int j = 0; j < 4; ++j) {
-        raw[j] = zs[j] - gzs[j];
-        act[j] = (ALLIN || pix[j] >= 0) && raw[j] >= -a.neg;
-        dn[j] = a.pos_over_neg;
-        any |= act[j];
-        if (!TSDF_LEAN_BAND) any_div |= act[j] && !(raw[j] > a.pos);
-      }
-      if (TSDF_LEAN_BAND) {
-        if (__builtin_fminf(__builtin_fminf(raw[0], raw[1]), __builtin_fminf(raw[2], raw[3])) <= a.pos) {
-#pragma unroll
-          for (int j = 0; j < 4; ++j) any_div |= act[j] && !(raw[j] > a.pos);
+      if (row_free) {
+#pragma unroll
+        for (int j = 0; j < 4; ++j) raw[j] = __builtin_inff(), act[j] = true, dn[j] = a.pos_over_neg;
+        any = true;
+      } else {
+#pragma unroll
+        for (int j = 0; j < 4; ++j) {
+          raw[j] = zs[j] - gzs[j];
+          act[j] = (ALLIN || pix[j] >= 0) && raw[j] >= -a.neg;
+          dn[j] = a.pos_over_neg;
+          any |= act[j];
+          if (!TSDF_LEAN_BAND) any_div |= act[j] && !(raw[j] > a.pos);
+        }
+        if (TSDF_LEAN_BAND) {
+          if (__builtin_fminf(__builtin_fminf(raw[0], raw[1]), __builtin_fminf(raw[2], raw[3])) <= a.pos) {
+#pragma unroll
+            for (int j = 0; j < 4; ++j) any_div |= act[j] && !(raw[j] > a.pos);
+          }
+        }
+      }
+      if constexpr (COUNT && ALLIN) {
+        if (a.db_mode == 2) {
+          if ((rcls & 3u) == TSDF_ROW_HIDDEN) {
+#pragma unroll
+            for (int j = 0; j < 4; ++j) n_viol += act[j] ? 1u : 0u;
+          }
+          if ((rcls & 3u) == TSDF_ROW_FREE) {
+            const uint2 bx = s_box[((unsigned)(ty + r * a.TY) << (a.log2TX - 6)) + (tid >> 6 & (unsigned)((a.TX >> 6) - 1))];
+#pragma unroll
+            for (int j = 0; j < 4; ++j) {
+              const unsigned pu = (unsigned)pix[j] % (unsigned)a.W, pv = (unsigned)pix[j] / (unsigned)a.W;
+              const bool inbox = pu >= (bx.x & 0xffffu) && pu <= bx.x >> 16 && pv >= (bx.y & 0xffffu) && pv <= bx.y >> 16;
+              n_viol += act[j] && raw[j] > a.pos && inbox ? 0u : 1u;
+            }
+          }
         }
       }
       if (COLOR) asm volatile("" ::"v"(cs[0]), "v"(cs[1]), "v"(cs[2]), "v"(cs[3]));
@@ -928,6 +1036,19 @@
       if (s_chg) atomicAdd(n_obs + 1024u + (b & 1023u), (unsigned long long)s_chg);
       if (s_imp) atomicAdd(n_obs + 2048u + (b & 1023u), (unsigned long long)s_imp);
       if (s_rdb) atomicAdd(n_obs + 3072u + (b & 1023u), (unsigned long long)s_rdb);
+    }
+    if constexpr (ALLIN) {
+      if (a.db_mode) {
+        unsigned long long *c = n_obs + 4096u;
+        const unsigned long long t_rows = __popcll(__builtin_amdgcn_ballot_w64(n_rows != 0u)), t_hid = __popcll(__builtin_amdgcn_ballot_w64(n_hid != 0u)),
+                                 t_fre = __popcll(__builtin_amdgcn_ballot_w64(n_fre != 0u));
+        if ((tid & 63u) == 0u) {
+          if (t_rows) atomicAdd(c + 0, t_rows);
+          if (t_hid) atomicAdd(c + 1, t_hid);
+          if (t_fre) atomicAdd(c + 2, t_fre);
+        }
+        if (n_viol) atomicAdd(c + 3, (unsigned long long)n_viol);
+      }
     }
   }
 }
@@ -1909,6 +2030,8 @@
   a.band_fy = h->band_fy;
   a.x_abs0 = a.y_abs0 = 0;
   a.zfast = 0;
+  a.db_mode = 0;
+  a.db_tab = nullptr;
   return hh;
 }
 
@@ -2300,6 +2423,7 @@
   const tsdf_params &p = h->p;
   h->count_slots = 0;
   h->count_ran = false;
+  h->db_mode_counted = 0;
   const IntegrateHost hh = make_args(h, T);
   IntegrateArgs a = hh.a;
   unsigned gx = (unsigned)((a.qpr + a.TX - 1) / a.TX);
@@ -2523,7 +2647,7 @@
       live = h->live;
     }
   }
-  if (count) TSDF_HIP_TRY(hipMemsetAsync(h->counter, 0, 4096 * sizeof(unsigned long long), h->stream));
+  if (count) TSDF_HIP_TRY(hipMemsetAsync(h->counter, 0, 4104 * sizeof(unsigned long long), h->stream));
   bool pose_ok = true;
   for (int i = 0; i < 12; ++i) pose_ok &= std::isfinite(T[i]) && fabsf(T[i]) <= 1e15f;
   const bool fastproj = fast_projection_ok(hh, p.integrate_color != 0);
@@ -2575,6 +2699,23 @@
   } while (0)
     const bool pipe = (tsdf_tuning().pipe & (color ? 2 : 1)) && fastproj && allin && !live && h->packed && a.hinge_fixed && a.neg_in_window &&
                       a.ny % a.TY == 0;
+    if (tsdf_tuning().depth_bounds && !pipe && fastproj && allin && !live && a.log2TX >= 6 && h->ctr_increasing[0] &&
+        a.W <= 8 * TSDF_DB_MAX_TW && a.H <= 65535 && a.W >= 1 && a.H >= 1) {
+      const size_t entries = tsdf_db_entries(a.W, a.H);
+      if (entries > h->db_cap) {
+        TSDF_HIP_TRY(hipStreamSynchronize(h->stream));
+        if (h->db_tab) TSDF_HIP_TRY(hipFree(h->db_tab));
+        h->db_tab = nullptr, h->db_cap = 0;
+        TSDF_HIP_TRY(hipMalloc(&h->db_tab, entries * sizeof(TsdfDB2)));
+        h->db_cap = entries;
+      }
+      const int tw = (a.W + 7) >> TSDF_DB_TILE_LOG2, th = (a.H + 7) >> TSDF_DB_TILE_LOG2;
+      hipLaunchKernelGGL(k_depth_bounds, dim3((unsigned)th), dim3(256), 0, h->stream, d_depth, a.W, a.H, tw, tsdf_db_levels(tw), h->db_tab);
+      TSDF_HIP_TRY(hipGetLastError());
+      a.db_mode = tsdf_tuning().depth_bounds == 2 ? 2 : 1;
+      a.db_tab = h->db_tab;
+      h->db_mode_counted = count ? a.db_mode : 0;
+    }
     if (pipe) {
       h->last_launch[0] |= 0x100;
 #define LAUNCH_P(ORDER, COUNT)                                                                                                           \
@@ -2644,20 +2785,27 @@
     tsdf_set_error("tsdf_integrate_collect without a counting launch");
     return TSDF_HIP_E_INVALID;
   }
-  unsigned long long c[4096];
+  unsigned long long c[4104];
   const int slots = h->count_slots;
-  TSDF_HIP_TRY(hipMemcpyAsync(c, h->counter, (size_t)slots * sizeof(unsigned long long), hipMemcpyDeviceToHost, h->stream));
+  const bool classes = h->db_mode_counted != 0 && slots == 4096;
+  TSDF_HIP_TRY(hipMemcpyAsync(c, h->counter, (size_t)(classes ? 4104 : slots) * sizeof(unsigned long long), hipMemcpyDeviceToHost, h->stream));
   TSDF_HIP_TRY(hipStreamSynchronize(h->stream));
   unsigned long long sum = 0, changed = 0, implied = 0, read_bytes = 0;
   for (int i = 0; i < 1024; ++i) sum += c[i];
   for (int i = 1024; i < slots && i < 2048; ++i) changed += c[i];
   for (int i = 2048; i < slots && i < 3072; ++i) implied += c[i];
-  for (int i = 3072; i < slots; ++i) read_bytes += c[i];
+  for (int i = 3072; i < slots && i < 4096; ++i) read_bytes += c[i];
   h->last_observed = h->count_ran ? sum : 0;
   h->last_changed_bytes = h->count_ran ? changed : 0;
   h->last_implied = h->count_ran ? implied : 0;
   h->last_read_bytes = h->count_ran ? read_bytes : 0;
   h->count_slots = 0;
+  for (int i = 0; i < 5; ++i) h->last_row_classes[i] = 0;
+  if (classes && h->count_ran) {
+    for (int i = 0; i < 4; ++i) h->last_row_classes[i] = c[4096 + i];
+    h->last_row_classes[4] = h->db_mode_counted == 1 ? 1 : 0;
+  }
+  h->db_mode_counted = 0;
   if (n_observed) *n_observed = h->last_observed;
   return TSDF_HIP_OK;
 }
@@ -2831,6 +2979,13 @@
   return TSDF_HIP_OK;
 }
 
+extern "C" int tsdf_hip_last_row_classes(tsdf_handle h, uint64_t out[5]) {
+  if (!h || !out) return TSDF_HIP_E_INVALID;
+  if (h->multi) return tsdf_multi_last_row_classes(h, out);
+  for (int i = 0; i < 5; ++i) out[i] = h->last_row_classes[i];
+  return TSDF_HIP_OK;
+}
+
 extern "C" int tsdf_hip_set_reference_cull(tsdf_handle h, const float planes[24]) {
   if (!h) return TSDF_HIP_E_INVALID;
   if (h->multi) return tsdf_multi_set_reference_cull(h, planes);
diff --git a/cpu_tsdf_amd/csrc/tsdf_multi.hip b/cpu_tsdf_amd/csrc/tsdf_multi.hip
--- a/cpu_tsdf_amd/csrc/tsdf_multi.hip
+++ b/cpu_tsdf_amd/csrc/tsdf_multi.hip
@@ -661,6 +661,16 @@
   return TSDF_HIP_OK;
 }
 
+int tsdf_multi_last_row_classes(tsdf_handle h, uint64_t out[5]) {
+  for (int i = 0; i < 4; ++i) out[i] = 0;
+  out[4] = 1;
+  for (tsdf_handle s : h->multi->slab) {
+    for (int i = 0; i < 4; ++i) out[i] += s->last_row_classes[i];
+    out[4] = out[4] && s->last_row_classes[4] ? 1 : 0;
+  }
+  return TSDF_HIP_OK;
+}
+
 int tsdf_multi_last_count_detail(tsdf_handle h, uint64_t out[2]) {
   out[0] = h->last_observed;
   out[1] = h->last_changed_bytes;
diff --git a/include/tsdf_hip.h b/include/tsdf_hip.h
--- a/include/tsdf_hip.h
+++ b/include/tsdf_hip.h
@@ -91,6 +91,7 @@
 
 int tsdf_hip_last_count_detail(tsdf_handle h, uint64_t out[2]);
 int tsdf_hip_last_read_detail(tsdf_handle h, uint64_t out[3]);
+int tsdf_hip_last_row_classes(tsdf_handle h, uint64_t out[5]);
 
 int tsdf_hip_set_weighting(tsdf_handle h, int weight_by_depth, int weight_by_variance);
 
```

Result: faster. 695,300, median of 6 (+4.3%).
